# Edward-Sun/DIFUSCO

Measured on NVIDIA H100. Metric: TSP-500 graphs/sec, 50-step categorical denoise, higher is better.
Workload: dtype f32 (3-term bf16 split on wgmma, fp32 accumulate)

## Files before the change

### difusco_b200/_cabi.py

```python
import ctypes as C
import os

import numpy as np

HERE = os.path.dirname(os.path.abspath(__file__))
LIB_PATH = os.path.join(HERE, "libdifusco_b200.so")

DFB_OK, DFB_E_INVALID, DFB_E_CUDA, DFB_E_UNSUPPORTED, DFB_E_NOMEM = 0, -1, -2, -3, -4
CATEGORICAL, GAUSSIAN = 0, 1
EDGE_IMPL_TC, EDGE_IMPL_FP32, EDGE_IMPL_TC1 = 0, 1, 2
AGGREGATION = {"sum": 0, "mean": 1, "max": 2}

SYMBOLS = [
    "dfb_abi_version", "dfb_create", "dfb_destroy", "dfb_last_error", "dfb_set_aggregation",
    "dfb_set_edge_impl", "dfb_load_weights", "dfb_prepare_graph", "dfb_prepare_graph_instances", "dfb_set_points",
    "dfb_encoder_forward", "dfb_denoise_step", "dfb_denoise", "dfb_denoise_record", "dfb_denoise_host",
    "dfb_launch_count", "dfb_profile_begin", "dfb_profile_end", "dfb_debug_edge_gemm", "dfb_debug_gnn_layer",
    "dfb_debug_phase_cycles", "dfb_debug_watchdog", "dfb_knn_graph", "dfb_set_graph_capture",
    "dfb_set_phase_timing", "dfb_tsp_merge_sparse", "dfb_tsp_merge_order", "dfb_two_opt", "dfb_write_heatmap_txt",
]

_lib = None


def lib():
  global _lib
  if _lib is not None:
    return _lib
  if not os.path.exists(LIB_PATH):
    raise RuntimeError(
        f"{LIB_PATH} not found: build it with `python -m difusco_b200.build` "
        "(difusco_b200 has no fallback path; the CUDA library is the product)")
  L = C.CDLL(LIB_PATH)
  vp, i32, i64, u64, f32 = C.c_void_p, C.c_int, C.c_int64, C.c_uint64, C.c_float
  L.dfb_abi_version.restype = i32
  L.dfb_create.argtypes = [C.POINTER(vp), i32]
  L.dfb_destroy.argtypes = [vp]
  L.dfb_last_error.argtypes = [vp]
  L.dfb_last_error.restype = C.c_char_p
  L.dfb_set_aggregation.argtypes = [vp, i32]
  L.dfb_set_edge_impl.argtypes = [vp, i32]
  L.dfb_load_weights.argtypes = [vp, i32, i32, i32, i32, i32, C.POINTER(C.c_char_p), C.POINTER(vp),
                                 C.POINTER(i64)]
  L.dfb_prepare_graph.argtypes = [vp, vp, i64, i64, i32, vp]
  L.dfb_prepare_graph_instances.argtypes = [vp, vp, i64, i64, i32, C.POINTER(i64), vp]
  L.dfb_set_points.argtypes = [vp, vp, vp]
  L.dfb_encoder_forward.argtypes = [vp, vp, f32, vp, vp]
  L.dfb_denoise_step.argtypes = [vp, i32, vp, f32, C.POINTER(f32), i32, vp, u64, i32, vp, vp, vp, vp]
  L.dfb_denoise.argtypes = [vp, i32, vp, i32, C.POINTER(C.c_int32), C.POINTER(f32),
                            C.POINTER(C.c_int32), vp, u64, vp]
  L.dfb_denoise_record.argtypes = [vp, i32, vp, i32, C.POINTER(C.c_int32), C.POINTER(f32), C.POINTER(C.c_int32), vp,
                                   u64, i32, C.POINTER(C.c_int32), vp, vp, vp, vp]
  L.dfb_denoise_host.argtypes = [vp, i32, vp, vp, i64, i64, i32, vp, i32, C.POINTER(C.c_int32),
                                 C.POINTER(f32), C.POINTER(C.c_int32), u64, vp, vp]
  L.dfb_launch_count.argtypes = [vp]
  L.dfb_launch_count.restype = i64
  L.dfb_profile_begin.argtypes = [vp]
  L.dfb_profile_end.argtypes = [vp, C.POINTER(C.c_double), C.POINTER(i64)]
  L.dfb_debug_edge_gemm.argtypes = [vp, i32, vp, vp, vp]
  L.dfb_debug_gnn_layer.argtypes = [vp, i32, f32, vp, vp, vp]
  L.dfb_debug_phase_cycles.argtypes = [vp, C.POINTER(C.c_uint64)]
  L.dfb_debug_watchdog.argtypes = [vp, C.POINTER(C.c_int)]
  L.dfb_set_graph_capture.argtypes = [vp, i32]
  L.dfb_set_phase_timing.argtypes = [vp, i32]
  L.dfb_knn_graph.argtypes = [vp, vp, i64, i32, i64, vp, vp]
  L.dfb_tsp_merge_sparse.argtypes = [vp, i64, vp, vp, i64, i32, vp, C.POINTER(i64)]
  L.dfb_tsp_merge_order.argtypes = [i64, vp, i64, vp, C.POINTER(i64)]
  L.dfb_two_opt.argtypes = [vp, vp, i64, vp, i64, i64, C.POINTER(i64), vp]
  L.dfb_write_heatmap_txt.argtypes = [C.c_char_p, i64, vp]
  for name in SYMBOLS:
    fn = getattr(L, name)
    if fn.restype is C.c_int and name not in ("dfb_abi_version",):
      fn.restype = i32
  _lib = L
  return L


class DfbError(RuntimeError):
  pass


def _raise(code, msg):
  msg = msg.decode() if isinstance(msg, bytes) else msg
  if code == DFB_E_INVALID:
    raise ValueError(msg)
  if code == DFB_E_UNSUPPORTED:
    raise NotImplementedError(msg)
  if code == DFB_E_NOMEM:
    raise MemoryError(msg)
  raise DfbError(msg)


MERGE_COMPLETE, MERGE_INCOMPLETE, MERGE_AMBIGUOUS = 0, 1, 2


def tsp_merge_sparse(points, heat, edge_index, mode=0):
  points = np.ascontiguousarray(points, dtype=np.float64)
  heat = np.ascontiguousarray(heat, dtype=np.float32).reshape(-1)
  edge_index = np.ascontiguousarray(edge_index, dtype=np.int64)
  n = points.shape[0]
  if edge_index.ndim != 2 or edge_index.shape[0] != 2 or edge_index.shape[1] != heat.shape[0]:
    raise ValueError("edge_index must be (2, E) with one heat value per edge")
  tour = np.empty(n + 1, dtype=np.int64)
  it = C.c_int64(0)
  rc = lib().dfb_tsp_merge_sparse(points.ctypes.data, n, heat.ctypes.data, edge_index.ctypes.data, heat.shape[0],
                                  int(mode), tour.ctypes.data, C.byref(it))
  if rc < 0:
    _raise(rc, "dfb_tsp_merge_sparse: invalid argument (n >= 3, indices inside [0, n), mode 0/1)")
  return rc, tour, it.value


def tsp_merge_order(n, order):
  order = np.ascontiguousarray(order, dtype=np.int64).reshape(-1)
  tour = np.empty(n + 1, dtype=np.int64)
  it = C.c_int64(0)
  rc = lib().dfb_tsp_merge_order(int(n), order.ctypes.data, order.shape[0], tour.ctypes.data, C.byref(it))
  if rc < 0:
    _raise(rc, "dfb_tsp_merge_order: invalid argument or the order does not complete a tour")
  return tour, it.value


def write_heatmap_txt(path, matrix):
  m = np.ascontiguousarray(matrix, dtype=np.float64)
  if m.ndim != 2 or m.shape[0] != m.shape[1]:
    raise ValueError("matrix must be square")
  rc = lib().dfb_write_heatmap_txt(os.fsencode(path), m.shape[0], m.ctypes.data)
  if rc != DFB_OK:
    _raise(rc, f"dfb_write_heatmap_txt: cannot write {path}")


_DEVICE_CTX = {}


def device_context(device_index, prefer=None):
  ctx = _DEVICE_CTX.get(device_index)
  if ctx is None or getattr(ctx, "_h", None) is None:
    ctx = prefer if prefer is not None else Context(device_index)
    _DEVICE_CTX[device_index] = ctx
  return ctx


class Context(object):

  def __init__(self, device=0):
    L = lib()
    h = C.c_void_p()
    rc = L.dfb_create(C.byref(h), int(device))
    if rc != DFB_OK:
      _raise(rc, L.dfb_last_error(None))
    self._h = h
    self.device = int(device)
    self._keep = []

  def close(self):
    if getattr(self, "_h", None):
      lib().dfb_destroy(self._h)
      self._h = None

  def __del__(self):
    try:
      self.close()
    except Exception:
      pass

  def _ck(self, rc):
    if rc != DFB_OK:
      _raise(rc, lib().dfb_last_error(self._h))

  def load_weights(self, state_dict, n_layers, hidden_dim, out_channels, node_feature_only, consts=None):
    items = [(k, np.ascontiguousarray(v, dtype=np.float32)) for k, v in state_dict.items()]
    for k, v in (consts or {}).items():
      items.append((k, np.ascontiguousarray(v, dtype=np.float32)))
    n = len(items)
    names = (C.c_char_p * n)(*[k.encode() for k, _ in items])
    ptrs = (C.c_void_p * n)(*[v.ctypes.data for _, v in items])
    numels = (C.c_int64 * n)(*[v.size for _, v in items])
    self._ck(lib().dfb_load_weights(self._h, n_layers, hidden_dim, out_channels, int(bool(node_feature_only)),
                                    n, names, ptrs, numels))

  def set_aggregation(self, name):
    if name not in AGGREGATION:
      raise ValueError(f"unknown aggregation {name}")
    self._ck(lib().dfb_set_aggregation(self._h, AGGREGATION[name]))

  def set_edge_impl(self, impl):
    self._ck(lib().dfb_set_edge_impl(self._h, impl))

  def prepare_graph(self, edge_index_ptr, num_nodes, num_edges, gn_segments=1, stream=0):
    self._ck(lib().dfb_prepare_graph(self._h, edge_index_ptr, num_nodes, num_edges, gn_segments, stream))

  def prepare_graph_instances(self, edge_index_ptr, num_nodes, num_edges, node_ptr, stream=0):
    node_ptr = np.ascontiguousarray(node_ptr, dtype=np.int64)
    self._ck(lib().dfb_prepare_graph_instances(self._h, edge_index_ptr, num_nodes, num_edges, node_ptr.size - 1,
                                               node_ptr.ctypes.data_as(C.POINTER(C.c_int64)), stream))

  def set_points(self, points_ptr, stream=0):
    self._ck(lib().dfb_set_points(self._h, points_ptr, stream))

  def encoder_forward(self, xt_ptr, t, out_ptr, stream=0):
    self._ck(lib().dfb_encoder_forward(self._h, xt_ptr, float(t), out_ptr, stream))

  def denoise_step(self, diffusion, xt_in_ptr, t, consts, last, uniforms_ptr, seed, step_index, xt_out_ptr,
                   p_out_ptr=None, net_out_ptr=None, stream=0):
    c = (C.c_float * 4)(*[float(x) for x in consts])
    self._ck(lib().dfb_denoise_step(self._h, diffusion, xt_in_ptr, float(t), c, int(last), uniforms_ptr,
                                    int(seed) & 0xFFFFFFFFFFFFFFFF, int(step_index), xt_out_ptr, p_out_ptr,
                                    net_out_ptr, stream))

  @staticmethod
  def _sched_arrays(t1, consts, last):
    steps = len(t1)
    t1a = (C.c_int32 * steps)(*[int(x) for x in t1])
    ca = (C.c_float * (4 * steps))(*[float(x) for row in consts for x in row])
    la = (C.c_int32 * steps)(*[int(x) for x in last])
    return steps, t1a, ca, la

  def denoise(self, diffusion, xt_ptr, t1, consts, last, uniforms_ptr=None, seed=0, stream=0):
    steps, t1a, ca, la = self._sched_arrays(t1, consts, last)
    self._ck(lib().dfb_denoise(self._h, diffusion, xt_ptr, steps, t1a, ca, la, uniforms_ptr,
                               int(seed) & 0xFFFFFFFFFFFFFFFF, stream))

  def denoise_record(self, diffusion, xt_ptr, t1, consts, last, record_steps, rec_xt_ptr=None, rec_p_ptr=None,
                     rec_out_ptr=None, uniforms_ptr=None, seed=0, stream=0):
    steps, t1a, ca, la = self._sched_arrays(t1, consts, last)
    n_rec = len(record_steps)
    ra = (C.c_int32 * max(n_rec, 1))(*[int(x) for x in record_steps])
    self._ck(lib().dfb_denoise_record(self._h, diffusion, xt_ptr, steps, t1a, ca, la, uniforms_ptr,
                                      int(seed) & 0xFFFFFFFFFFFFFFFF, n_rec, ra, rec_xt_ptr, rec_p_ptr, rec_out_ptr,
                                      stream))

  def denoise_host(self, diffusion, points_ptr, edge_index_ptr, num_nodes, num_edges, gn_segments, xt0_ptr,
                   t1, consts, last, seed, heatmap_ptr, stream=0):
    steps, t1a, ca, la = self._sched_arrays(t1, consts, last)
    self._ck(lib().dfb_denoise_host(self._h, diffusion, points_ptr, edge_index_ptr, num_nodes, num_edges,
                                    gn_segments, xt0_ptr, steps, t1a, ca, la,
                                    int(seed) & 0xFFFFFFFFFFFFFFFF, heatmap_ptr, stream))

  def two_opt(self, points, tours, max_iterations, stream=0):
    points = np.ascontiguousarray(points, dtype=np.float64)
    tours = np.array(tours, dtype=np.int64, order="C", copy=True)
    if tours.ndim != 2 or tours.shape[1] != points.shape[0] + 1:
      raise ValueError("tours must be (batch, n + 1)")
    it = C.c_int64(0)
    self._ck(lib().dfb_two_opt(self._h, points.ctypes.data, points.shape[0], tours.ctypes.data, tours.shape[0],
                               int(max_iterations), C.byref(it), stream))
    return tours, it.value

  def knn_graph(self, points_ptr, num_nodes, k, node_offset, edge_index_ptr, stream=0):
    self._ck(lib().dfb_knn_graph(self._h, points_ptr, int(num_nodes), int(k), int(node_offset), edge_index_ptr, stream))

  def launch_count(self):
    return int(lib().dfb_launch_count(self._h))

  def profile_begin(self):
    self._ck(lib().dfb_profile_begin(self._h))

  def profile_end(self):
    ms, n = C.c_double(0), C.c_int64(0)
    self._ck(lib().dfb_profile_end(self._h, C.byref(ms), C.byref(n)))
    return ms.value, n.value

  def set_graph_capture(self, enabled):
    self._ck(lib().dfb_set_graph_capture(self._h, int(bool(enabled))))

  def debug_watchdog(self):
    out = (C.c_int * 4)()
    lib().dfb_debug_watchdog(self._h, out)
    return [int(x) for x in out]

  def set_phase_timing(self, enabled):
    self._ck(lib().dfb_set_phase_timing(self._h, int(bool(enabled))))

  def debug_phase_cycles(self):
    out = (C.c_uint64 * 32)()
    self._ck(lib().dfb_debug_phase_cycles(self._h, out))
    return [int(x) for x in out]

  def debug_edge_gemm(self, layer, e_in_ptr, acc_out_ptr, stream=0):
    self._ck(lib().dfb_debug_edge_gemm(self._h, layer, e_in_ptr, acc_out_ptr, stream))

  def debug_gnn_layer(self, layer, t, h_ptr, e_ptr, stream=0):
    self._ck(lib().dfb_debug_gnn_layer(self._h, int(layer), float(t), h_ptr, e_ptr, stream))
```

### difusco_b200/csrc/dfb_api.cu

```cuda
#include <cuda_runtime.h>
#include <math.h>
#include <stdio.h>
#include <stdlib.h>
#include <string.h>

#include <map>
#include <string>
#include <vector>

#include "../../include/difusco_b200.h"
#include "common.cuh"
#include "edge_layer_fp32.cuh"
#include "edge_layer_tc.cuh"
#include "kernels_small.cuh"
#include "knn.cuh"
#include "tsp_decode.cuh"

using namespace dfb;

static std::string g_create_error;

struct DevBuf {
  void* p = nullptr;
  size_t cap = 0;
  DevBuf() = default;
  DevBuf(const DevBuf&) = delete;
  DevBuf& operator=(const DevBuf&) = delete;
  ~DevBuf() { if (p) cudaFree(p); }
};

struct dfb_ctx {
  int device = 0;
  std::string err;
  bool weights_loaded = false;
  int L = 0, out_channels = 0, node_only = 0;
  int agg_mode = AGG_SUM;
  int edge_impl = DFB_EDGE_IMPL_TC;
  bool phase_timing = false;
  DevBuf wbuf, wbuf16, layers_dev;
  std::vector<LayerParams> layers;
  TimeParams tp{};
  HeadParams hp{};
  const float *Wt_node = nullptr, *b_node = nullptr, *Wt_edge = nullptr, *b_edge = nullptr;
  const float *dimt128 = nullptr, *dimt256 = nullptr;
  float* lut = nullptr;
  bool graph_ready = false, points_ready = false;
  GraphDev g{};
  GnSegments gseg{};
  int gn_blocks = 0;
  DevBuf d_row, d_col, d_perm, d_rowptr, d_grp_first, d_grp_pair, d_ei_stage, d_seg_start, d_seg_blk_first, d_gn_blk;
  DevBuf e, h, h0, uvab, uvab0, partials, feat, tvec, tvals, gn_part, gn_stats, d_points, d_xt, d_u;
  DevBuf opt_points, opt_tours, opt_pos, opt_dnext, opt_cand, opt_tiles, opt_state, opt_best;
  int tvec_steps_cap = 0;
  static constexpr int STAGE_SLOTS = 2, MAX_STEPS = 4096;
  float* h_tvals[STAGE_SLOTS] = {nullptr, nullptr};
  StepParams* h_steps[STAGE_SLOTS] = {nullptr, nullptr};
  cudaEvent_t stage_ev[STAGE_SLOTS] = {nullptr, nullptr};
  int stage_next = 0;
  DevBuf d_steps;
  uint64_t buf_gen = 0;
  bool capture_enabled = true;
  bool capture_broken = false;
  cudaGraphExec_t loop_exec = nullptr;
  cudaStream_t loop_stream = nullptr;
  cudaEvent_t loop_in = nullptr, loop_out = nullptr;
  struct LoopKey {
    uint64_t buf_gen = ~0ull;
    int steps = 0, diffusion = 0, impl = 0, agg = 0;
    bool timed = false;
    const void* uniforms = nullptr;
    bool operator==(const LoopKey& o) const {
      return buf_gen == o.buf_gen && steps == o.steps && diffusion == o.diffusion && impl == o.impl && agg == o.agg &&
             timed == o.timed && uniforms == o.uniforms;
    }
  } loop_key;
  int64_t loop_launches = 0;
  int64_t launches = 0;
  bool profiling = false;
  std::vector<cudaEvent_t> ev_pool;
  size_t ev_used = 0;
  TcState tc;

  ~dfb_ctx() {
    for (cudaEvent_t ev : ev_pool) cudaEventDestroy(ev);
    if (loop_exec) cudaGraphExecDestroy(loop_exec);
    if (loop_stream) cudaStreamDestroy(loop_stream);
    if (loop_in) cudaEventDestroy(loop_in);
    if (loop_out) cudaEventDestroy(loop_out);
    for (int i = 0; i < STAGE_SLOTS; ++i) {
      if (h_tvals[i]) cudaFreeHost(h_tvals[i]);
      if (h_steps[i]) cudaFreeHost(h_steps[i]);
      if (stage_ev[i]) cudaEventDestroy(stage_ev[i]);
    }
  }
};

#define FAIL(ctx, code, ...)                         \
  do {                                               \
    char _b[512];                                    \
    snprintf(_b, sizeof(_b), __VA_ARGS__);           \
    (ctx)->err = _b;                                 \
    return (code);                                   \
  } while (0)

#define CK(ctx, call)                                                                       \
  do {                                                                                      \
    cudaError_t _e = (call);                                                                \
    if (_e != cudaSuccess)                                                                  \
      FAIL(ctx, DFB_E_CUDA, "%s failed: %s (%s:%d)", #call, cudaGetErrorString(_e), __FILE__, __LINE__); \
  } while (0)

#define CKL(ctx)                                                                           \
  do {                                                                                      \
    (ctx)->launches++;                                                                      \
    cudaError_t _e = cudaGetLastError();                                                    \
    if (_e != cudaSuccess)                                                                  \
      FAIL(ctx, DFB_E_CUDA, "kernel launch failed: %s (%s:%d)", cudaGetErrorString(_e), __FILE__, __LINE__); \
  } while (0)

static int ensure(dfb_ctx* ctx, DevBuf& b, size_t bytes) {
  if (bytes <= b.cap) return DFB_OK;
  ctx->buf_gen++;
  if (b.p) cudaFree(b.p);
  b.p = nullptr;
  b.cap = 0;
  size_t want = bytes + (bytes >> 3);
  cudaError_t e = cudaMalloc(&b.p, want);
  if (e != cudaSuccess) {
    e = cudaMalloc(&b.p, bytes);
    want = bytes;
  }
  if (e != cudaSuccess) {
    cudaGetLastError();
    FAIL(ctx, DFB_E_NOMEM, "cudaMalloc(%zu bytes) failed: %s", bytes, cudaGetErrorString(e));
  }
  b.cap = want;
  return DFB_OK;
}
#define ENS(ctx, buf, bytes)                     \
  do {                                           \
    int _r = ensure(ctx, buf, bytes);            \
    if (_r) return _r;                           \
  } while (0)

static bool is_device_ptr(const void* p) {
  cudaPointerAttributes a;
  if (cudaPointerGetAttributes(&a, p) != cudaSuccess) {
    cudaGetLastError();
    return false;
  }
  return a.type == cudaMemoryTypeDevice || a.type == cudaMemoryTypeManaged;
}

extern "C" int dfb_abi_version(void) { return DFB_ABI_VERSION; }

extern "C" const char* dfb_last_error(const dfb_ctx* ctx) {
  return ctx ? ctx->err.c_str() : g_create_error.c_str();
}

extern "C" int dfb_create(dfb_ctx** out, int device) {
  if (!out) return DFB_E_INVALID;
  *out = nullptr;
  int n = 0;
  cudaError_t e = cudaGetDeviceCount(&n);
  if (e != cudaSuccess || n == 0) {
    g_create_error = std::string("no CUDA device: ") + cudaGetErrorString(e) +
                     " (difusco_b200 has no CPU fallback)";
    cudaGetLastError();
    return DFB_E_CUDA;
  }
  if (device < 0 || device >= n) {
    g_create_error = "device index out of range";
    return DFB_E_INVALID;
  }
  if ((e = cudaSetDevice(device)) != cudaSuccess) {
    g_create_error = std::string("cudaSetDevice: ") + cudaGetErrorString(e);
    return DFB_E_CUDA;
  }
  cudaDeviceProp prop;
  cudaGetDeviceProperties(&prop, device);
  if (prop.major != 9 || prop.minor != 0) {
    char b[160];
    snprintf(b, sizeof(b), "device %d is sm_%d%d; this library is built for sm_90a (H100) only", device,
             prop.major, prop.minor);
    g_create_error = b;
    return DFB_E_UNSUPPORTED;
  }
  dfb_ctx* ctx = new dfb_ctx();
  ctx->device = device;
  e = cudaFuncSetAttribute(k_edge_layer_fp32, cudaFuncAttributeMaxDynamicSharedMemorySize, EF_SMEM);
  if (e != cudaSuccess) {
    g_create_error = std::string("cudaFuncSetAttribute(fp32 edge kernel): ") + cudaGetErrorString(e);
    delete ctx;
    return DFB_E_CUDA;
  }
  int r = tc_init(&ctx->tc, prop.multiProcessorCount);
  if (r != 0) {
    g_create_error = "tensor-core edge kernel setup failed: " + ctx->tc.err;
    delete ctx;
    return DFB_E_CUDA;
  }
  for (int i = 0; i < dfb_ctx::STAGE_SLOTS; ++i) {
    if ((e = cudaHostAlloc((void**)&ctx->h_tvals[i], dfb_ctx::MAX_STEPS * sizeof(float), cudaHostAllocDefault)) != cudaSuccess ||
        (e = cudaHostAlloc((void**)&ctx->h_steps[i], dfb_ctx::MAX_STEPS * sizeof(StepParams), cudaHostAllocDefault)) != cudaSuccess ||
        (e = cudaEventCreateWithFlags(&ctx->stage_ev[i], cudaEventDisableTiming)) != cudaSuccess) {
      g_create_error = std::string("pinned staging: ") + cudaGetErrorString(e);
      delete ctx;
      return DFB_E_CUDA;
    }
  }
  if ((e = cudaStreamCreateWithFlags(&ctx->loop_stream, cudaStreamNonBlocking)) != cudaSuccess ||
      (e = cudaEventCreateWithFlags(&ctx->loop_in, cudaEventDisableTiming)) != cudaSuccess ||
      (e = cudaEventCreateWithFlags(&ctx->loop_out, cudaEventDisableTiming)) != cudaSuccess) {
    g_create_error = std::string("loop stream: ") + cudaGetErrorString(e);
    delete ctx;
    return DFB_E_CUDA;
  }
  {
    const char* cg = getenv("DFB_GRAPH_CAPTURE");
    if (cg && atoi(cg) == 0) ctx->capture_enabled = false;
  }
  *out = ctx;
  return DFB_OK;
}

extern "C" int dfb_destroy(dfb_ctx* ctx) {
  if (!ctx) return DFB_OK;
  cudaSetDevice(ctx->device);
  delete ctx;
  return DFB_OK;
}

extern "C" int dfb_set_edge_impl(dfb_ctx* ctx, int impl) {
  if (!ctx) return DFB_E_INVALID;
  if (impl != DFB_EDGE_IMPL_TC && impl != DFB_EDGE_IMPL_FP32 && impl != DFB_EDGE_IMPL_TC1) FAIL(ctx, DFB_E_INVALID, "unknown edge impl %d", impl);
  ctx->edge_impl = impl;
  return DFB_OK;
}

extern "C" int64_t dfb_launch_count(const dfb_ctx* ctx) { return ctx ? ctx->launches : 0; }

static uint16_t f2bf16_rn(float f) {
  uint32_t u;
  memcpy(&u, &f, 4);
  if ((u & 0x7fffffffu) > 0x7f800000u) return (uint16_t)((u >> 16) | 0x40);
  uint32_t r = u + 0x7fffu + ((u >> 16) & 1u);
  return (uint16_t)(r >> 16);
}
static float bf16_to_f(uint16_t h) {
  uint32_t u = (uint32_t)h << 16;
  float f;
  memcpy(&f, &u, 4);
  return f;
}

extern "C" int dfb_load_weights(dfb_ctx* ctx, int n_layers, int hidden_dim, int out_channels,
                                int node_feature_only, int n_tensors, const char* const* names,
                                const float* const* tensors, const int64_t* numels) {
  if (!ctx) return DFB_E_INVALID;
  CK(ctx, cudaSetDevice(ctx->device));
  if (hidden_dim != H) FAIL(ctx, DFB_E_UNSUPPORTED, "hidden_dim %d: kernels are specialised for 256", hidden_dim);
  if (n_layers < 1 || n_layers > 64) FAIL(ctx, DFB_E_INVALID, "n_layers %d out of range", n_layers);
  if (out_channels != 1 && out_channels != 2) FAIL(ctx, DFB_E_INVALID, "out_channels must be 1 or 2");
  std::map<std::string, std::pair<const float*, int64_t>> sd;
  for (int i = 0; i < n_tensors; ++i) {
    std::string k = names[i];
    if (k.rfind("model.", 0) == 0) k = k.substr(6);
    sd[k] = {tensors[i], numels[i]};
  }
  auto get = [&](const std::string& k, int64_t n, const float** out) -> int {
    auto it = sd.find(k);
    if (it == sd.end()) FAIL(ctx, DFB_E_INVALID, "state_dict key '%s' missing", k.c_str());
    if (it->second.second != n)
      FAIL(ctx, DFB_E_INVALID, "state_dict key '%s' has %lld elements, expected %lld", k.c_str(),
           (long long)it->second.second, (long long)n);
    *out = it->second.first;
    return DFB_OK;
  };
#define GET(k, n, out)                 \
  do {                                 \
    int _r = get(k, n, out);           \
    if (_r) return _r;                 \
  } while (0)

  const int L = n_layers;
  std::vector<float> arena;
  auto put = [&](size_t n) {
    size_t off = arena.size();
    arena.resize(off + ((n + 63) / 64) * 64, 0.0f);
    return off;
  };
  auto put_T = [&](const float* W, int out_f, int in_f) {
    size_t off = put((size_t)out_f * in_f);
    for (int o = 0; o < out_f; ++o)
      for (int i = 0; i < in_f; ++i) arena[off + (size_t)i * out_f + o] = W[(size_t)o * in_f + i];
    return off;
  };
  auto put_v = [&](const float* v, int n) {
    size_t off = put(n);
    memcpy(&arena[off], v, n * sizeof(float));
    return off;
  };
  struct LOff {
    size_t Wt_uvab, b_uvab, Wt_C, Wt_O, b_O, hg, hb, eg, eb, og, ob, Wt_tau, b_tau;
  };
  std::vector<LOff> lo(L);
  std::vector<uint16_t> arena16((size_t)w_arena_rows(L) * H);
  auto put16 = [&](const float* W, int row) {
    uint16_t* hi = &arena16[(size_t)row * H];
    for (int i = 0; i < H * H; ++i) {
      hi[i] = f2bf16_rn(W[i]);
      hi[W_LO_ROWS * H + i] = f2bf16_rn(W[i] - bf16_to_f(hi[i]));
    }
  };
  const float* p;
  for (int l = 0; l < L; ++l) {
    std::string pre = "layers." + std::to_string(l) + ".";
    const float *W[4], *b[4], *WC, *bC;
    const char* nm[4] = {"U", "V", "A", "B"};
    for (int q = 0; q < 4; ++q) {
      GET(pre + nm[q] + ".weight", H * H, &W[q]);
      GET(pre + nm[q] + ".bias", H, &b[q]);
    }
    GET(pre + "C.weight", H * H, &WC);
    GET(pre + "C.bias", H, &bC);
    lo[l].Wt_uvab = put((size_t)H * 4 * H);
    lo[l].b_uvab = put(4 * H);
    for (int q = 0; q < 4; ++q) {
      for (int o = 0; o < H; ++o) {
        for (int i = 0; i < H; ++i) arena[lo[l].Wt_uvab + (size_t)i * 4 * H + q * H + o] = W[q][(size_t)o * H + i];
        arena[lo[l].b_uvab + q * H + o] = b[q][o] + (q == 3 ? bC[o] : 0.0f);
      }
    }
    lo[l].Wt_C = put_T(WC, H, H);
    GET(pre + "norm_h.weight", H, &p); lo[l].hg = put_v(p, H);
    GET(pre + "norm_h.bias", H, &p);   lo[l].hb = put_v(p, H);
    GET(pre + "norm_e.weight", H, &p); lo[l].eg = put_v(p, H);
    GET(pre + "norm_e.bias", H, &p);   lo[l].eb = put_v(p, H);
    std::string po = "per_layer_out." + std::to_string(l) + ".";
    const float* WO;
    GET(po + "0.weight", H, &p); lo[l].og = put_v(p, H);
    GET(po + "0.bias", H, &p);   lo[l].ob = put_v(p, H);
    GET(po + "2.weight", H * H, &WO); lo[l].Wt_O = put_T(WO, H, H);
    GET(po + "2.bias", H, &p);   lo[l].b_O = put_v(p, H);
    std::string pt = "time_embed_layers." + std::to_string(l) + ".1.";
    GET(pt + "weight", H * TE, &p); lo[l].Wt_tau = put_T(p, H, TE);
    GET(pt + "bias", H, &p);        lo[l].b_tau = put_v(p, H);
    put16(WC, w_row_C(l));
    put16(WO, w_row_O(l));
    for (int q = 0; q < 4; ++q) put16(W[q], w_row_UVAB(l) + q * W_MAT_ROWS);
  }
  size_t o_node_W, o_node_b, o_edge_W, o_edge_b, o_t0W, o_t0b, o_t2W, o_t2b, o_gng, o_gnb, o_outW, o_outb;
  GET("node_embed.weight", H * H, &p); o_node_W = put_T(p, H, H); put16(p, w_row_embed(L, 1));
  GET("node_embed.bias", H, &p);       o_node_b = put_v(p, H);
  GET("edge_embed.weight", H * H, &p); o_edge_W = put_T(p, H, H); put16(p, w_row_embed(L, 0));
  GET("edge_embed.bias", H, &p);       o_edge_b = put_v(p, H);
  GET("time_embed.0.weight", TE * H, &p); o_t0W = put_T(p, TE, H);
  GET("time_embed.0.bias", TE, &p);       o_t0b = put_v(p, TE);
  GET("time_embed.2.weight", TE * TE, &p); o_t2W = put_T(p, TE, TE);
  GET("time_embed.2.bias", TE, &p);        o_t2b = put_v(p, TE);
  GET("out.0.weight", H, &p); o_gng = put_v(p, H);
  GET("out.0.bias", H, &p);   o_gnb = put_v(p, H);
  GET("out.2.weight", out_channels * H, &p); o_outW = put_v(p, out_channels * H);
  GET("out.2.bias", out_channels, &p);       o_outb = put_v(p, out_channels);

  size_t o_freqs = put(TE), o_d128 = put(TE), o_d256 = put(H), o_lut = put(2 * H);
  auto it = sd.find("__const.time_freqs");
  for (int m = 0; m < TE; ++m)
    arena[o_freqs + m] = (it != sd.end() && it->second.second == TE)
                             ? it->second.first[m]
                             : expf((-9.210340371976184f * (float)m) / (float)TE);
  it = sd.find("__const.dimt_pos");
  for (int m = 0; m < TE; ++m)
    arena[o_d128 + m] = (it != sd.end() && it->second.second == TE)
                            ? it->second.first[m]
                            : powf(10000.0f, (2.0f * (float)(m / 2)) / (float)TE);
  it = sd.find("__const.dimt_scalar");
  for (int m = 0; m < H; ++m)
    arena[o_d256 + m] = (it != sd.end() && it->second.second == H)
                            ? it->second.first[m]
                            : powf(10000.0f, (2.0f * (float)(m / 2)) / (float)H);

  ENS(ctx, ctx->wbuf, arena.size() * sizeof(float));
  ENS(ctx, ctx->wbuf16, arena16.size() * sizeof(uint16_t));
  ENS(ctx, ctx->layers_dev, L * sizeof(LayerParams));
  CK(ctx, cudaMemcpy(ctx->wbuf.p, arena.data(), arena.size() * sizeof(float), cudaMemcpyHostToDevice));
  CK(ctx, cudaMemcpy(ctx->wbuf16.p, arena16.data(), arena16.size() * sizeof(uint16_t), cudaMemcpyHostToDevice));
  const float* base = (const float*)ctx->wbuf.p;
  ctx->layers.resize(L);
  for (int l = 0; l < L; ++l) {
    LayerParams& lp = ctx->layers[l];
    lp.Wt_uvab = base + lo[l].Wt_uvab; lp.b_uvab = base + lo[l].b_uvab;
    lp.Wt_C = base + lo[l].Wt_C; lp.Wt_O = base + lo[l].Wt_O; lp.b_O = base + lo[l].b_O;
    lp.ln_h_g = base + lo[l].hg; lp.ln_h_b = base + lo[l].hb;
    lp.ln_e_g = base + lo[l].eg; lp.ln_e_b = base + lo[l].eb;
    lp.ln_o_g = base + lo[l].og; lp.ln_o_b = base + lo[l].ob;
    lp.Wt_tau = base + lo[l].Wt_tau; lp.b_tau = base + lo[l].b_tau;
  }
  CK(ctx, cudaMemcpy(ctx->layers_dev.p, ctx->layers.data(), L * sizeof(LayerParams), cudaMemcpyHostToDevice));
  ctx->Wt_node = base + o_node_W; ctx->b_node = base + o_node_b;
  ctx->Wt_edge = base + o_edge_W; ctx->b_edge = base + o_edge_b;
  ctx->tp.freqs = base + o_freqs; ctx->tp.Wt0 = base + o_t0W; ctx->tp.b0 = base + o_t0b;
  ctx->tp.Wt2 = base + o_t2W;     ctx->tp.b2 = base + o_t2b;
  ctx->hp.gn_g = base + o_gng; ctx->hp.gn_b = base + o_gnb; ctx->hp.W = base + o_outW; ctx->hp.b = base + o_outb;
  ctx->hp.out_channels = out_channels;
  ctx->dimt128 = base + o_d128; ctx->dimt256 = base + o_d256;
  ctx->lut = (float*)ctx->wbuf.p + o_lut;
  ctx->L = L; ctx->out_channels = out_channels; ctx->node_only = node_feature_only;

  int r = tc_bind_weights(&ctx->tc, (const uint16_t*)ctx->wbuf16.p, L);
  if (r) FAIL(ctx, DFB_E_CUDA, "tensor-map setup failed: %s", ctx->tc.err.c_str());

  if (!node_feature_only) {
    ENS(ctx, ctx->feat, (size_t)LIN_ROWS * H * sizeof(float));
    float x01[2] = {0.0f, 1.0f};
    ENS(ctx, ctx->tvals, 4096 * sizeof(float));
    CK(ctx, cudaMemcpy(ctx->tvals.p, x01, sizeof(x01), cudaMemcpyHostToDevice));
    k_scalar_features<<<2, H>>>((const float*)ctx->tvals.p, nullptr, ctx->dimt256, (float*)ctx->feat.p, 2);
    CKL(ctx);
    k_linear<<<dim3(1, 1), 256>>>((const float*)ctx->feat.p, ctx->Wt_edge, ctx->b_edge, ctx->lut, 2, H);
    CKL(ctx);
    CK(ctx, cudaDeviceSynchronize());
  }
  ctx->weights_loaded = true;
  ctx->buf_gen++;
  ctx->points_ready = false;
  return DFB_OK;
}

extern "C" int dfb_set_aggregation(dfb_ctx* ctx, int mode) {
  if (!ctx) return DFB_E_INVALID;
  if (mode < AGG_SUM || mode > AGG_MAX) FAIL(ctx, DFB_E_INVALID, "unknown aggregation %d", mode);
  ctx->agg_mode = mode;
  return DFB_OK;
}

static int prepare_graph(dfb_ctx* ctx, const int64_t* edge_index, int64_t V64, int64_t E64, int gn_segments,
                         int n_inst, const int64_t* node_ptr, cudaStream_t st) {
  if (!ctx) return DFB_E_INVALID;
  CK(ctx, cudaSetDevice(ctx->device));
  if (!ctx->weights_loaded) FAIL(ctx, DFB_E_INVALID, "dfb_load_weights must be called first");
  if (V64 <= 0 || E64 <= 0 || V64 > 0x7fffffff / 4 || E64 > 0x7ffffff0)
    FAIL(ctx, DFB_E_INVALID, "bad graph size V=%lld E=%lld", (long long)V64, (long long)E64);
  const int V = (int)V64, E = (int)E64;
  const int R = ctx->node_only ? V : E;
  if (!node_ptr) {
    if (gn_segments < 1) FAIL(ctx, DFB_E_INVALID, "gn_segments must be >= 1");
    if (R % gn_segments) FAIL(ctx, DFB_E_INVALID, "gn_segments %d does not divide %d rows", gn_segments, R);
  } else {
    if (n_inst < 1) FAIL(ctx, DFB_E_INVALID, "n_instances %d < 1", n_inst);
    if (node_ptr[0] != 0 || node_ptr[n_inst] != V64)
      FAIL(ctx, DFB_E_INVALID, "node_ptr must run from 0 to num_nodes %lld (got %lld .. %lld)", (long long)V64,
           (long long)node_ptr[0], (long long)node_ptr[n_inst]);
    for (int i = 0; i < n_inst; ++i)
      if (node_ptr[i + 1] <= node_ptr[i])
        FAIL(ctx, DFB_E_INVALID, "node_ptr must be strictly increasing (instance %d: %lld after %lld)", i,
             (long long)node_ptr[i + 1], (long long)node_ptr[i]);
  }
  std::vector<int64_t> stage;
  const int64_t* ei = edge_index;
  if (is_device_ptr(edge_index)) {
    stage.resize((size_t)2 * E);
    CK(ctx, cudaMemcpyAsync(stage.data(), edge_index, (size_t)2 * E * sizeof(int64_t), cudaMemcpyDeviceToHost, st));
    CK(ctx, cudaStreamSynchronize(st));
    ei = stage.data();
  }
  const int64_t* row64 = ei;
  const int64_t* col64 = ei + E;
  std::vector<int> inst;
  if (node_ptr) {
    inst.resize(V);
    for (int i = 0; i < n_inst; ++i)
      for (int64_t v = node_ptr[i]; v < node_ptr[i + 1]; ++v) inst[v] = i;
  }
  std::vector<int> rowptr((size_t)V + 1, 0);
  bool sorted = true;
  for (int s = 0; s < E; ++s) {
    int64_t r = row64[s], c = col64[s];
    if (r < 0 || r >= V || c < 0 || c >= V)
      FAIL(ctx, DFB_E_INVALID, "edge %d = (%lld,%lld) out of range for %d nodes", s, (long long)r, (long long)c, V);
    if (node_ptr && inst[r] != inst[c])
      FAIL(ctx, DFB_E_INVALID, "edge %d = (%lld,%lld) joins instances %d and %d", s, (long long)r, (long long)c,
           inst[r], inst[c]);
    rowptr[(size_t)r + 1]++;
    if (s && r < row64[s - 1]) sorted = false;
  }
  for (int i = 0; i < V; ++i) rowptr[i + 1] += rowptr[i];
  const int S = node_ptr ? n_inst : gn_segments;
  std::vector<int> seg_start((size_t)S + 1), blk_first((size_t)S + 1);
  for (int i = 0; i <= S; ++i) {
    if (!node_ptr) seg_start[i] = (int)((int64_t)R / S * i);
    else seg_start[i] = ctx->node_only ? (int)node_ptr[i] : rowptr[node_ptr[i]];
  }
  for (int i = 0; i < S; ++i)
    if (seg_start[i + 1] == seg_start[i])
      FAIL(ctx, DFB_E_INVALID, "instance %d (nodes %lld..%lld) has no edges: its GroupNorm would be over zero rows", i,
           (long long)node_ptr[i], (long long)node_ptr[i + 1] - 1);
  std::vector<int2> gn_blk;
  for (int i = 0; i < S; ++i) {
    blk_first[i] = (int)gn_blk.size();
    for (int r0 = seg_start[i]; r0 < seg_start[i + 1]; r0 += GN_ROWS_PER_BLOCK) gn_blk.push_back(make_int2(i, r0));
  }
  blk_first[S] = (int)gn_blk.size();
  const int nb = (int)gn_blk.size();

  std::vector<int> row(E), col(E), perm;
  if (sorted) {
    for (int s = 0; s < E; ++s) {
      row[s] = (int)row64[s];
      col[s] = (int)col64[s];
    }
  } else {
    perm.resize(E);
    std::vector<int> cur(rowptr.begin(), rowptr.end() - 1);
    for (int s = 0; s < E; ++s) {
      int pos = cur[row64[s]]++;
      perm[pos] = s;
      row[pos] = (int)row64[s];
      col[pos] = (int)col64[s];
    }
  }
  const int nG = (E + GROUP - 1) / GROUP;
  std::vector<int> gfirst(nG), gpair((size_t)nG + 1);
  int np = 0;
  for (int gI = 0; gI < nG; ++gI) {
    int s0 = gI * GROUP, s1 = std::min(E, s0 + GROUP) - 1;
    gfirst[gI] = row[s0];
    gpair[gI] = np;
    np += row[s1] - row[s0] + 1;
  }
  gpair[nG] = np;

  ENS(ctx, ctx->d_row, (size_t)E * 4);
  ENS(ctx, ctx->d_col, (size_t)E * 4);
  ENS(ctx, ctx->d_rowptr, ((size_t)V + 1) * 4);
  ENS(ctx, ctx->d_grp_first, (size_t)nG * 4);
  ENS(ctx, ctx->d_grp_pair, ((size_t)nG + 1) * 4);
  CK(ctx, cudaMemcpyAsync(ctx->d_row.p, row.data(), (size_t)E * 4, cudaMemcpyHostToDevice, st));
  CK(ctx, cudaMemcpyAsync(ctx->d_col.p, col.data(), (size_t)E * 4, cudaMemcpyHostToDevice, st));
  CK(ctx, cudaMemcpyAsync(ctx->d_rowptr.p, rowptr.data(), ((size_t)V + 1) * 4, cudaMemcpyHostToDevice, st));
  CK(ctx, cudaMemcpyAsync(ctx->d_grp_first.p, gfirst.data(), (size_t)nG * 4, cudaMemcpyHostToDevice, st));
  CK(ctx, cudaMemcpyAsync(ctx->d_grp_pair.p, gpair.data(), ((size_t)nG + 1) * 4, cudaMemcpyHostToDevice, st));
  if (!sorted) {
    ENS(ctx, ctx->d_perm, (size_t)E * 4);
    CK(ctx, cudaMemcpyAsync(ctx->d_perm.p, perm.data(), (size_t)E * 4, cudaMemcpyHostToDevice, st));
  }
  ENS(ctx, ctx->d_seg_start, ((size_t)S + 1) * 4);
  ENS(ctx, ctx->d_seg_blk_first, ((size_t)S + 1) * 4);
  ENS(ctx, ctx->d_gn_blk, (size_t)nb * sizeof(int2));
  CK(ctx, cudaMemcpyAsync(ctx->d_seg_start.p, seg_start.data(), ((size_t)S + 1) * 4, cudaMemcpyHostToDevice, st));
  CK(ctx, cudaMemcpyAsync(ctx->d_seg_blk_first.p, blk_first.data(), ((size_t)S + 1) * 4, cudaMemcpyHostToDevice, st));
  CK(ctx, cudaMemcpyAsync(ctx->d_gn_blk.p, gn_blk.data(), (size_t)nb * sizeof(int2), cudaMemcpyHostToDevice, st));
  CK(ctx, cudaStreamSynchronize(st));
  GraphDev& g = ctx->g;
  g.V = V; g.E = E;
  g.row = (const int*)ctx->d_row.p; g.col = (const int*)ctx->d_col.p;
  g.perm = sorted ? nullptr : (const int*)ctx->d_perm.p;
  g.rowptr = (const int*)ctx->d_rowptr.p;
  g.n_groups = nG; g.grp_first = (const int*)ctx->d_grp_first.p; g.grp_pair = (const int*)ctx->d_grp_pair.p;
  g.n_pairs = np;
  ctx->gseg.n_segs = S;
  ctx->gseg.start = (const int*)ctx->d_seg_start.p;
  ctx->gseg.blk_first = (const int*)ctx->d_seg_blk_first.p;
  ctx->gseg.blk = (const int2*)ctx->d_gn_blk.p;
  ctx->gn_blocks = nb;

  ENS(ctx, ctx->e, (size_t)E * H * sizeof(float));
  ENS(ctx, ctx->h, (size_t)V * H * sizeof(float));
  ENS(ctx, ctx->h0, (size_t)V * H * sizeof(float));
  ENS(ctx, ctx->uvab, (size_t)V * 4 * H * sizeof(float));
  ENS(ctx, ctx->uvab0, (size_t)V * 4 * H * sizeof(float));
  ENS(ctx, ctx->partials, (size_t)np * H * sizeof(float));
  const size_t feat_rows = 65536;
  ENS(ctx, ctx->feat, feat_rows * H * sizeof(float));
  ENS(ctx, ctx->gn_part, std::max((size_t)nb, (size_t)1024) * 32 * 2 * sizeof(double));
  ENS(ctx, ctx->gn_stats, (size_t)S * 32 * 2 * sizeof(float));
  ENS(ctx, ctx->d_xt, (size_t)std::max(V, E) * sizeof(float));
  ctx->graph_ready = true;
  ctx->buf_gen++;
  ctx->points_ready = false;
  return DFB_OK;
}

extern "C" int dfb_prepare_graph(dfb_ctx* ctx, const int64_t* edge_index, int64_t num_nodes, int64_t num_edges,
                                 int gn_segments, void* stream) {
  return prepare_graph(ctx, edge_index, num_nodes, num_edges, gn_segments, 0, nullptr, (cudaStream_t)stream);
}

extern "C" int dfb_prepare_graph_instances(dfb_ctx* ctx, const int64_t* edge_index, int64_t num_nodes,
                                           int64_t num_edges, int n_instances, const int64_t* node_ptr, void* stream) {
  if (ctx && !node_ptr) FAIL(ctx, DFB_E_INVALID, "node_ptr is required");
  return prepare_graph(ctx, edge_index, num_nodes, num_edges, 0, n_instances, node_ptr, (cudaStream_t)stream);
}

struct EdgeImpl { bool fp32; int nwg; };
static EdgeImpl edge_impl(const dfb_ctx* ctx) {
  return {ctx->edge_impl == DFB_EDGE_IMPL_FP32, ctx->edge_impl == DFB_EDGE_IMPL_TC1 ? 1 : 2};
}

static int linear_rows(dfb_ctx* ctx, const float* X, const float* Wt, int w_row, const float* b, float* Y, int R, int N,
                       cudaStream_t st) {
  if (edge_impl(ctx).fp32) {
    dim3 grid((R + LIN_ROWS - 1) / LIN_ROWS, N / 256);
    k_linear<<<grid, 256, 0, st>>>(X, Wt, b, Y, R, N);
    CKL(ctx);
    return DFB_OK;
  }
  if (tc_launch_linear(&ctx->tc, X, Y, b, R, N / H, w_row, st))
    FAIL(ctx, DFB_E_CUDA, "tensor-core linear: %s", ctx->tc.err.c_str());
  ctx->launches++;
  return DFB_OK;
}

static int node_linears(dfb_ctx* ctx, int l, const float* h, float* uvab, int V, cudaStream_t st) {
  const LayerParams& lp = ctx->layers[l];
  return linear_rows(ctx, h, lp.Wt_uvab, w_row_UVAB(l), lp.b_uvab, uvab, V, 4 * H, st);
}

static int embed_rows(dfb_ctx* ctx, int which, const float* X, float* Y, int R, cudaStream_t st) {
  return linear_rows(ctx, X, which ? ctx->Wt_node : ctx->Wt_edge, w_row_embed(ctx->L, which),
                     which ? ctx->b_node : ctx->b_edge, Y, R, H, st);
}

extern "C" int dfb_set_points(dfb_ctx* ctx, const float* points, void* stream_) {
  if (!ctx) return DFB_E_INVALID;
  cudaStream_t st = (cudaStream_t)stream_;
  CK(ctx, cudaSetDevice(ctx->device));
  if (!ctx->graph_ready) FAIL(ctx, DFB_E_INVALID, "dfb_prepare_graph must be called first");
  if (ctx->node_only) FAIL(ctx, DFB_E_INVALID, "dfb_set_points is for the TSP encoder (node_feature_only=0)");
  const int V = ctx->g.V;
  const float* dp = points;
  if (!is_device_ptr(points)) {
    ENS(ctx, ctx->d_points, (size_t)V * 2 * sizeof(float));
    CK(ctx, cudaMemcpyAsync(ctx->d_points.p, points, (size_t)V * 2 * sizeof(float), cudaMemcpyHostToDevice, st));
    dp = (const float*)ctx->d_points.p;
  }
  const int CH = 65536;
  for (int v0 = 0; v0 < V; v0 += CH) {
    int n = std::min(CH, V - v0);
    k_pos_features<<<n, H, 0, st>>>(dp + (size_t)v0 * 2, ctx->dimt128, (float*)ctx->feat.p, n);
    CKL(ctx);
    int r = embed_rows(ctx, 1, (const float*)ctx->feat.p, (float*)ctx->h0.p + (size_t)v0 * H, n, st);
    if (r) return r;
  }
  int r = node_linears(ctx, 0, (const float*)ctx->h0.p, (float*)ctx->uvab0.p, V, st);
  if (r) return r;
  ctx->points_ready = true;
  return DFB_OK;
}

static int launch_edge_layer(dfb_ctx* ctx, int l, float* e, const float* uvab, const float* tvec_edge, int write_e,
                             int e_zero, const float* xt_for_lut, cudaStream_t st) {
  cudaEvent_t ev0 = nullptr, ev1 = nullptr;
  if (ctx->profiling) {
    if (ctx->ev_used + 2 > ctx->ev_pool.size()) {
      for (int i = 0; i < 256; ++i) {
        cudaEvent_t ev;
        CK(ctx, cudaEventCreate(&ev));
        ctx->ev_pool.push_back(ev);
      }
    }
    ev0 = ctx->ev_pool[ctx->ev_used++];
    ev1 = ctx->ev_pool[ctx->ev_used++];
    CK(ctx, cudaEventRecord(ev0, st));
  }
  const EdgeImpl impl = edge_impl(ctx);
  if (impl.fp32) {
    if (e_zero) CK(ctx, cudaMemsetAsync(e, 0, (size_t)ctx->g.E * H * sizeof(float), st));
    if (xt_for_lut) {
      k_lut_expand<<<(ctx->g.E + 3) / 4, 256, 0, st>>>(xt_for_lut, ctx->g.perm, ctx->lut, e, ctx->g.E);
      CKL(ctx);
    }
    k_edge_layer_fp32<<<ctx->g.n_groups, 256, EF_SMEM, st>>>(e, uvab, (float*)ctx->partials.p,
                                                            ctx->g, ctx->layers[l], tvec_edge, write_e,
                                                            ctx->agg_mode);
    CKL(ctx);
  } else {
    if (tc_launch_edge_layer(&ctx->tc, l, e, uvab, (float*)ctx->partials.p, ctx->g, ctx->layers[l],
                             tvec_edge, write_e, e_zero, xt_for_lut, ctx->lut, ctx->agg_mode, impl.nwg,
                             ctx->phase_timing, nullptr, st))
      FAIL(ctx, DFB_E_CUDA, "tensor-core edge layer: %s", ctx->tc.err.c_str());
    ctx->launches++;
  }
  if (ctx->profiling) CK(ctx, cudaEventRecord(ev1, st));
  return DFB_OK;
}

static int run_layer(dfb_ctx* ctx, int l, float* h, float* e, const float* uv0, const float* tv, int e_zero,
                     const float* xt_lut, cudaStream_t st) {
  const int L = ctx->L;
  const float* uv = uv0;
  if (!uv) {
    int r = node_linears(ctx, l, h, (float*)ctx->uvab.p, ctx->g.V, st);
    if (r) return r;
    uv = (const float*)ctx->uvab.p;
  }
  const int write_e = !(ctx->node_only && l == L - 1);
  int r = launch_edge_layer(ctx, l, e, uv, ctx->node_only ? nullptr : tv, write_e, e_zero, xt_lut, st);
  if (r) return r;
  if (ctx->node_only || l < L - 1) {
    k_node_update<<<(ctx->g.V + 7) / 8, 256, 0, st>>>(h, uv, (const float*)ctx->partials.p, ctx->g,
                                                      ctx->layers[l].ln_h_g, ctx->layers[l].ln_h_b,
                                                      ctx->node_only ? tv : nullptr, ctx->agg_mode);
    CKL(ctx);
  }
  return DFB_OK;
}

static int run_forward(dfb_ctx* ctx, const float* xt, const float* tvec, bool binary_xt, PosteriorArgs pa,
                       cudaStream_t st) {
  const GraphDev& g = ctx->g;
  const int V = g.V, E = g.E;
  float* h = (float*)ctx->h.p;
  float* e = (float*)ctx->e.p;
  const float* xt_lut = nullptr;
  int e_zero = 0;
  if (!ctx->node_only) {
    if (!ctx->points_ready) FAIL(ctx, DFB_E_INVALID, "dfb_set_points must be called before a TSP forward");
    CK(ctx, cudaMemcpyAsync(h, ctx->h0.p, (size_t)V * H * sizeof(float), cudaMemcpyDeviceToDevice, st));
    if (binary_xt) {
      xt_lut = xt;
    } else {
      const int CH = 65536;
      for (int s0 = 0; s0 < E; s0 += CH) {
        int n = std::min(CH, E - s0);
        k_scalar_features<<<n, H, 0, st>>>(g.perm ? xt : xt + s0, g.perm ? g.perm + s0 : nullptr, ctx->dimt256,
                                           (float*)ctx->feat.p, n);
        CKL(ctx);
        int r = embed_rows(ctx, 0, (const float*)ctx->feat.p, e + (size_t)s0 * H, n, st);
        if (r) return r;
      }
    }
  } else {
    const int CH = 65536;
    for (int v0 = 0; v0 < V; v0 += CH) {
      int n = std::min(CH, V - v0);
      k_scalar_features<<<n, H, 0, st>>>(xt + v0, nullptr, ctx->dimt256, (float*)ctx->feat.p, n);
      CKL(ctx);
      int r = embed_rows(ctx, 1, (const float*)ctx->feat.p, h + (size_t)v0 * H, n, st);
      if (r) return r;
    }
    e_zero = 1;
  }
  for (int l = 0; l < ctx->L; ++l) {
    const bool first = l == 0;
    int r = run_layer(ctx, l, h, e, (first && !ctx->node_only) ? (const float*)ctx->uvab0.p : nullptr,
                      tvec + (size_t)l * H, first ? e_zero : 0, first ? xt_lut : nullptr, st);
    if (r) return r;
  }
  const float* Z = ctx->node_only ? h : e;
  const int R = ctx->node_only ? V : E;
  k_gn_partial<<<ctx->gn_blocks, 256, 0, st>>>(Z, ctx->gseg, (double*)ctx->gn_part.p);
  CKL(ctx);
  k_gn_final<<<dim3(ctx->gseg.n_segs, 32), 256, 0, st>>>((const double*)ctx->gn_part.p, Z, ctx->gseg,
                                                         (float*)ctx->gn_stats.p);
  CKL(ctx);
  k_head<<<(R + 255) / 256, 256, 0, st>>>(Z, R, ctx->gseg, (const float*)ctx->gn_stats.p,
                                      ctx->node_only ? nullptr : g.perm, ctx->hp, pa);
  CKL(ctx);
  return DFB_OK;
}

static int stage_acquire(dfb_ctx* ctx, int* slot) {
  *slot = ctx->stage_next;
  ctx->stage_next = (ctx->stage_next + 1) % dfb_ctx::STAGE_SLOTS;
  CK(ctx, cudaEventSynchronize(ctx->stage_ev[*slot]));
  return DFB_OK;
}

static int compute_tvecs(dfb_ctx* ctx, int slot, int S, cudaStream_t st) {
  ENS(ctx, ctx->tvals, std::max<size_t>(4096, (size_t)S) * sizeof(float));
  ENS(ctx, ctx->tvec, (size_t)S * ctx->L * H * sizeof(float));
  CK(ctx, cudaMemcpyAsync(ctx->tvals.p, ctx->h_tvals[slot], (size_t)S * sizeof(float), cudaMemcpyHostToDevice, st));
  k_time_vectors<<<S, 256, 0, st>>>((const float*)ctx->tvals.p, ctx->tp, (const LayerParams*)ctx->layers_dev.p,
                                    ctx->L, (float*)ctx->tvec.p);
  CKL(ctx);
  return DFB_OK;
}

extern "C" int dfb_encoder_forward(dfb_ctx* ctx, const float* xt, float t, float* out, void* stream_) {
  if (!ctx) return DFB_E_INVALID;
  cudaStream_t st = (cudaStream_t)stream_;
  CK(ctx, cudaSetDevice(ctx->device));
  if (!ctx->graph_ready) FAIL(ctx, DFB_E_INVALID, "dfb_prepare_graph must be called first");
  int slot;
  int r = stage_acquire(ctx, &slot);
  if (r) return r;
  ctx->h_tvals[slot][0] = t;
  r = compute_tvecs(ctx, slot, 1, st);
  if (r) return r;
  CK(ctx, cudaEventRecord(ctx->stage_ev[slot], st));
  PosteriorArgs pa{};
  pa.mode = HEAD_FORWARD;
  pa.net_out = out;
  return run_forward(ctx, xt, (const float*)ctx->tvec.p, false, pa, st);
}

static int step_args(dfb_ctx* ctx, int diffusion_type, const float* consts, int last, PosteriorArgs* pa) {
  if (diffusion_type == DFB_DIFFUSION_CATEGORICAL) {
    if (ctx->out_channels != 2) FAIL(ctx, DFB_E_INVALID, "categorical diffusion needs out_channels == 2");
    pa->mode = HEAD_CATEGORICAL;
  } else if (diffusion_type == DFB_DIFFUSION_GAUSSIAN) {
    if (ctx->out_channels != 1) FAIL(ctx, DFB_E_INVALID, "gaussian diffusion needs out_channels == 1");
    pa->mode = HEAD_GAUSSIAN;
  } else {
    FAIL(ctx, DFB_E_INVALID, "Unknown diffusion type %d", diffusion_type);
  }
  if (consts)
    for (int i = 0; i < 4; ++i) pa->c[i] = consts[i];
  pa->last = last;
  return DFB_OK;
}

extern "C" int dfb_denoise_step(dfb_ctx* ctx, int diffusion_type, const float* xt_in, float t,
                                const float* consts, int last, const float* uniforms, uint64_t seed,
                                int step_index, float* xt_out, float* p_out, float* net_out, void* stream_) {
  if (!ctx) return DFB_E_INVALID;
  cudaStream_t st = (cudaStream_t)stream_;
  CK(ctx, cudaSetDevice(ctx->device));
  if (!ctx->graph_ready) FAIL(ctx, DFB_E_INVALID, "dfb_prepare_graph must be called first");
  PosteriorArgs pa{};
  int r = step_args(ctx, diffusion_type, consts, last, &pa);
  if (r) return r;
  int slot;
  r = stage_acquire(ctx, &slot);
  if (r) return r;
  ctx->h_tvals[slot][0] = t;
  r = compute_tvecs(ctx, slot, 1, st);
  if (r) return r;
  CK(ctx, cudaEventRecord(ctx->stage_ev[slot], st));
  pa.xt_in = xt_in; pa.uniforms = uniforms; pa.seed = seed; pa.step = (unsigned)step_index;
  pa.xt_out = xt_out; pa.p_out = p_out; pa.net_out = net_out;
  return run_forward(ctx, xt_in, (const float*)ctx->tvec.p, diffusion_type == DFB_DIFFUSION_CATEGORICAL, pa, st);
}

static int enqueue_loop(dfb_ctx* ctx, int diffusion_type, float* xt, int steps, const float* uniforms, cudaStream_t st) {
  const size_t N = ctx->node_only ? ctx->g.V : ctx->g.E;
  for (int i = 0; i < steps; ++i) {
    PosteriorArgs pa{};
    int r = step_args(ctx, diffusion_type, nullptr, 0, &pa);
    if (r) return r;
    pa.sp = (const StepParams*)ctx->d_steps.p + i;
    pa.xt_in = xt; pa.xt_out = xt;
    pa.uniforms = uniforms ? uniforms + (size_t)i * N : nullptr;
    r = run_forward(ctx, xt, (const float*)ctx->tvec.p + (size_t)i * ctx->L * H,
                    diffusion_type == DFB_DIFFUSION_CATEGORICAL, pa, st);
    if (r) return r;
  }
  return DFB_OK;
}

extern "C" int dfb_denoise(dfb_ctx* ctx, int diffusion_type, float* xt, int steps, const int32_t* t1,
                           const float* consts, const int32_t* last_flags, const float* uniforms,
                           uint64_t seed, void* stream_) {
  return dfb_denoise_record(ctx, diffusion_type, xt, steps, t1, consts, last_flags, uniforms, seed, 0, nullptr,
                            nullptr, nullptr, nullptr, stream_);
}

extern "C" int dfb_denoise_record(dfb_ctx* ctx, int diffusion_type, float* xt, int steps, const int32_t* t1,
                                  const float* consts, const int32_t* last_flags, const float* uniforms,
                                  uint64_t seed, int n_record, const int32_t* record_steps, float* rec_xt,
                                  float* rec_p, float* rec_out, void* stream_) {
  if (!ctx) return DFB_E_INVALID;
  cudaStream_t st = (cudaStream_t)stream_;
  CK(ctx, cudaSetDevice(ctx->device));
  if (!ctx->graph_ready) FAIL(ctx, DFB_E_INVALID, "dfb_prepare_graph must be called first");
  if (steps < 1 || steps > dfb_ctx::MAX_STEPS) FAIL(ctx, DFB_E_INVALID, "steps %d out of range", steps);
  if (!ctx->node_only && !ctx->points_ready) FAIL(ctx, DFB_E_INVALID, "dfb_set_points must be called before a TSP forward");
  {
    PosteriorArgs chk{};
    int r = step_args(ctx, diffusion_type, nullptr, 0, &chk);
    if (r) return r;
  }
  if (n_record < 0) FAIL(ctx, DFB_E_INVALID, "n_record %d < 0", n_record);
  if (n_record > 0) {
    if (!record_steps) FAIL(ctx, DFB_E_INVALID, "n_record > 0 needs record_steps");
    if (!rec_xt && !rec_p && !rec_out) FAIL(ctx, DFB_E_INVALID, "n_record > 0 with no record buffer");
    if (rec_p && diffusion_type != DFB_DIFFUSION_CATEGORICAL)
      FAIL(ctx, DFB_E_INVALID, "rec_p is the categorical posterior: not defined for gaussian diffusion");
    for (int j = 0; j < n_record; ++j) {
      if (record_steps[j] < 0 || record_steps[j] >= steps)
        FAIL(ctx, DFB_E_INVALID, "record step %d outside [0, %d)", record_steps[j], steps);
      if (j > 0 && record_steps[j] <= record_steps[j - 1])
        FAIL(ctx, DFB_E_INVALID, "record steps must be strictly increasing (%d after %d)", record_steps[j],
             record_steps[j - 1]);
    }
  }
  int slot;
  int r = stage_acquire(ctx, &slot);
  if (r) return r;
  const size_t N = ctx->node_only ? ctx->g.V : ctx->g.E;
  for (int i = 0, j = 0; i < steps; ++i) {
    ctx->h_tvals[slot][i] = (float)t1[i];
    StepParams& sp = ctx->h_steps[slot][i];
    for (int k = 0; k < 4; ++k) sp.c[k] = consts[4 * i + k];
    sp.last = last_flags[i];
    sp.step = (unsigned)i;
    sp.seed = seed;
    sp.rec_xt = sp.rec_p = sp.rec_out = nullptr;
    if (j < n_record && record_steps[j] == i) {
      if (rec_xt) sp.rec_xt = rec_xt + (size_t)j * N;
      if (rec_p) sp.rec_p = rec_p + (size_t)j * N;
      if (rec_out) sp.rec_out = rec_out + (size_t)j * N * ctx->out_channels;
      ++j;
    }
  }
  ENS(ctx, ctx->d_steps, (size_t)dfb_ctx::MAX_STEPS * sizeof(StepParams));
  r = compute_tvecs(ctx, slot, steps, st);
  if (r) return r;
  CK(ctx, cudaMemcpyAsync(ctx->d_steps.p, ctx->h_steps[slot], (size_t)steps * sizeof(StepParams), cudaMemcpyHostToDevice, st));
  CK(ctx, cudaEventRecord(ctx->stage_ev[slot], st));
  float* x = (float*)ctx->d_xt.p;
  if (xt != x) CK(ctx, cudaMemcpyAsync(x, xt, N * sizeof(float), cudaMemcpyDeviceToDevice, st));

  const bool want_graph = ctx->capture_enabled && !ctx->capture_broken && !ctx->profiling;
  if (want_graph) {
    dfb_ctx::LoopKey key;
    key.buf_gen = ctx->buf_gen; key.steps = steps; key.diffusion = diffusion_type; key.impl = ctx->edge_impl;
    key.agg = ctx->agg_mode; key.timed = ctx->phase_timing; key.uniforms = uniforms;
    if (!ctx->loop_exec || !(ctx->loop_key == key)) {
      if (ctx->loop_exec) {
        cudaGraphExecDestroy(ctx->loop_exec);
        ctx->loop_exec = nullptr;
      }
      const int64_t l0 = ctx->launches;
      cudaGraph_t graph = nullptr;
      cudaError_t ce = cudaStreamBeginCapture(ctx->loop_stream, cudaStreamCaptureModeThreadLocal);
      if (ce == cudaSuccess) {
        r = enqueue_loop(ctx, diffusion_type, x, steps, uniforms, ctx->loop_stream);
        ce = cudaStreamEndCapture(ctx->loop_stream, &graph);
        if (r == DFB_OK && ce == cudaSuccess) ce = cudaGraphInstantiate(&ctx->loop_exec, graph, 0);
        if (graph) cudaGraphDestroy(graph);
      }
      ctx->loop_launches = ctx->launches - l0;
      ctx->launches = l0;
      if (r != DFB_OK || ce != cudaSuccess || !ctx->loop_exec) {
        cudaGetLastError();
        ctx->loop_exec = nullptr;
        ctx->capture_broken = true;
        if (r != DFB_OK) return r;
      } else {
        ctx->loop_key = key;
      }
    }
  }
  if (want_graph && ctx->loop_exec) {
    CK(ctx, cudaEventRecord(ctx->loop_in, st));
    CK(ctx, cudaStreamWaitEvent(ctx->loop_stream, ctx->loop_in, 0));
    CK(ctx, cudaGraphLaunch(ctx->loop_exec, ctx->loop_stream));
    CK(ctx, cudaEventRecord(ctx->loop_out, ctx->loop_stream));
    CK(ctx, cudaStreamWaitEvent(st, ctx->loop_out, 0));
    ctx->launches += ctx->loop_launches;
  } else {
    r = enqueue_loop(ctx, diffusion_type, x, steps, uniforms, st);
    if (r) return r;
  }
  if (xt != x) CK(ctx, cudaMemcpyAsync(xt, x, N * sizeof(float), cudaMemcpyDeviceToDevice, st));
  return DFB_OK;
}

extern "C" int dfb_set_graph_capture(dfb_ctx* ctx, int enabled) {
  if (!ctx) return DFB_E_INVALID;
  ctx->capture_enabled = enabled != 0;
  ctx->capture_broken = false;
  return DFB_OK;
}

extern "C" int dfb_set_phase_timing(dfb_ctx* ctx, int enabled) {
  if (!ctx) return DFB_E_INVALID;
  ctx->phase_timing = enabled != 0;
  return DFB_OK;
}

extern "C" int dfb_denoise_host(dfb_ctx* ctx, int diffusion_type, const float* points,
                                const int64_t* edge_index, int64_t V, int64_t E, int gn_segments,
                                const float* xt0, int steps, const int32_t* t1, const float* consts,
                                const int32_t* last_flags, uint64_t seed, float* heatmap_out, void* stream_) {
  if (!ctx) return DFB_E_INVALID;
  cudaStream_t st = (cudaStream_t)stream_;
  CK(ctx, cudaSetDevice(ctx->device));
  int r = dfb_prepare_graph(ctx, edge_index, V, E, gn_segments, st);
  if (r) return r;
  if (!ctx->node_only) {
    if (!points) FAIL(ctx, DFB_E_INVALID, "points required for TSP");
    r = dfb_set_points(ctx, points, st);
    if (r) return r;
  }
  const size_t N = ctx->node_only ? (size_t)V : (size_t)E;
  CK(ctx, cudaMemcpyAsync(ctx->d_xt.p, xt0, N * sizeof(float), cudaMemcpyHostToDevice, st));
  r = dfb_denoise(ctx, diffusion_type, (float*)ctx->d_xt.p, steps, t1, consts, last_flags, nullptr, seed, st);
  if (r) return r;
  CK(ctx, cudaMemcpyAsync(heatmap_out, ctx->d_xt.p, N * sizeof(float), cudaMemcpyDeviceToHost, st));
  CK(ctx, cudaStreamSynchronize(st));
  return DFB_OK;
}

extern "C" int dfb_profile_begin(dfb_ctx* ctx) {
  if (!ctx) return DFB_E_INVALID;
  ctx->profiling = true;
  ctx->ev_used = 0;
  return DFB_OK;
}
extern "C" int dfb_profile_end(dfb_ctx* ctx, double* ms, int64_t* n) {
  if (!ctx) return DFB_E_INVALID;
  CK(ctx, cudaSetDevice(ctx->device));
  CK(ctx, cudaDeviceSynchronize());
  double tot = 0.0;
  for (size_t i = 0; i + 1 < ctx->ev_used; i += 2) {
    float t = 0.f;
    CK(ctx, cudaEventElapsedTime(&t, ctx->ev_pool[i], ctx->ev_pool[i + 1]));
    tot += t;
  }
  if (ms) *ms = tot;
  if (n) *n = (int64_t)(ctx->ev_used / 2);
  ctx->profiling = false;
  ctx->ev_used = 0;
  return DFB_OK;
}

extern "C" int dfb_debug_edge_gemm(dfb_ctx* ctx, int layer, const float* e_in, float* acc_out, void* stream_) {
  if (!ctx) return DFB_E_INVALID;
  cudaStream_t st = (cudaStream_t)stream_;
  CK(ctx, cudaSetDevice(ctx->device));
  if (!ctx->graph_ready) FAIL(ctx, DFB_E_INVALID, "dfb_prepare_graph must be called first");
  if (layer < 0 || layer >= ctx->L) FAIL(ctx, DFB_E_INVALID, "layer out of range");
  if (tc_launch_edge_layer(&ctx->tc, layer, const_cast<float*>(e_in), (const float*)ctx->uvab.p,
                           (float*)ctx->partials.p, ctx->g, ctx->layers[layer], nullptr, 0, 0, nullptr, ctx->lut, AGG_SUM,
                           edge_impl(ctx).nwg, false, acc_out, st))
    FAIL(ctx, DFB_E_CUDA, "tensor-core edge layer: %s", ctx->tc.err.c_str());
  ctx->launches++;
  return DFB_OK;
}

extern "C" int dfb_debug_gnn_layer(dfb_ctx* ctx, int layer, float t, float* h, float* e, void* stream_) {
  if (!ctx) return DFB_E_INVALID;
  cudaStream_t st = (cudaStream_t)stream_;
  CK(ctx, cudaSetDevice(ctx->device));
  if (!ctx->graph_ready) FAIL(ctx, DFB_E_INVALID, "dfb_prepare_graph must be called first");
  if (layer < 0 || layer >= ctx->L) FAIL(ctx, DFB_E_INVALID, "layer %d out of range for %d layers", layer, ctx->L);
  if (!is_device_ptr(h) || !is_device_ptr(e)) FAIL(ctx, DFB_E_INVALID, "h and e must be device pointers");
  int slot;
  int r = stage_acquire(ctx, &slot);
  if (r) return r;
  ctx->h_tvals[slot][0] = t;
  r = compute_tvecs(ctx, slot, 1, st);
  if (r) return r;
  CK(ctx, cudaEventRecord(ctx->stage_ev[slot], st));
  return run_layer(ctx, layer, h, e, nullptr, (const float*)ctx->tvec.p + (size_t)layer * H, 0, nullptr, st);
}

extern "C" int dfb_debug_phase_cycles(dfb_ctx* ctx, unsigned long long* out) {
  if (!ctx || !out) return DFB_E_INVALID;
  CK(ctx, cudaSetDevice(ctx->device));
  CK(ctx, cudaDeviceSynchronize());
  CK(ctx, cudaMemcpy(out, ctx->tc.phase_cycles, 32 * sizeof(unsigned long long), cudaMemcpyDeviceToHost));
  CK(ctx, cudaMemset(ctx->tc.phase_cycles, 0, 32 * sizeof(unsigned long long)));
  return DFB_OK;
}

extern "C" int dfb_debug_watchdog(dfb_ctx* ctx, int* out) {
  if (!ctx || !out || !ctx->tc.error_host) return DFB_E_INVALID;
  for (int i = 0; i < 4; ++i) out[i] = ((volatile int*)ctx->tc.error_host)[i];
  return DFB_OK;
}

extern "C" int dfb_knn_graph(dfb_ctx* ctx, const double* points, int64_t num_nodes, int k, int64_t node_offset,
                             int64_t* edge_index, void* stream_) {
  if (!ctx) return DFB_E_INVALID;
  cudaStream_t st = (cudaStream_t)stream_;
  CK(ctx, cudaSetDevice(ctx->device));
  if (num_nodes < 1 || k < 1 || k > num_nodes) FAIL(ctx, DFB_E_INVALID, "bad kNN size N=%lld K=%d", (long long)num_nodes, k);
  if ((size_t)num_nodes * sizeof(double) > 200 * 1024) FAIL(ctx, DFB_E_UNSUPPORTED, "kNN graph: N=%lld exceeds the shared-memory brute-force limit (25600)", (long long)num_nodes);
  const size_t smem = (size_t)num_nodes * sizeof(double) + (size_t)(num_nodes + 31) / 32 * sizeof(unsigned);
  if (!is_device_ptr(edge_index)) FAIL(ctx, DFB_E_INVALID, "edge_index must be a device pointer");
  const double* dp = points;
  if (!is_device_ptr(points)) {
    for (int64_t i = 0; i < 2 * num_nodes; ++i)
      if (!std::isfinite(points[i])) FAIL(ctx, DFB_E_INVALID, "kNN graph: non-finite coordinate of node %lld", (long long)(i / 2));
    ENS(ctx, ctx->d_points, (size_t)num_nodes * 2 * sizeof(double));
    CK(ctx, cudaMemcpyAsync(ctx->d_points.p, points, (size_t)num_nodes * 2 * sizeof(double), cudaMemcpyHostToDevice, st));
    dp = (const double*)ctx->d_points.p;
  }
  CK(ctx, cudaFuncSetAttribute(k_knn_bruteforce, cudaFuncAttributeMaxDynamicSharedMemorySize, (int)smem));
  k_knn_bruteforce<<<(int)num_nodes, 256, smem, st>>>(dp, (int)num_nodes, k, (long long*)edge_index, (long long)node_offset);
  CKL(ctx);
  return DFB_OK;
}

extern "C" int dfb_tsp_merge_sparse(const double* points, int64_t n, const float* heat, const int64_t* edge_index, int64_t E,
                                    int mode, int64_t* tour, int64_t* merge_iterations) {
  if (!points || !heat || !edge_index || !tour || !merge_iterations || n < 3 || n > 0x7fffffff / 2 || E < 0 || (mode != 0 && mode != 1))
    return DFB_E_INVALID;
  int r = tspmerge::merge_sparse(points, (int)n, heat, edge_index, E, mode, tour, merge_iterations);
  return r < 0 ? DFB_E_INVALID : r;
}

extern "C" int dfb_tsp_merge_order(int64_t n, const int64_t* order, int64_t count, int64_t* tour, int64_t* merge_iterations) {
  if (!order || !tour || !merge_iterations || n < 3 || n > 0x7fffffff / 2 || count < 0) return DFB_E_INVALID;
  int r = tspmerge::merge_order((int)n, order, count, tour, merge_iterations);
  return r < 0 ? DFB_E_INVALID : r;
}

extern "C" int dfb_two_opt(dfb_ctx* ctx, const double* points, int64_t n, int64_t* tours, int64_t batch, int64_t max_iterations,
                           int64_t* iterations_out, void* stream_) {
  if (!ctx) return DFB_E_INVALID;
  cudaStream_t st = (cudaStream_t)stream_;
  CK(ctx, cudaSetDevice(ctx->device));
  if (!points || !tours || !iterations_out) FAIL(ctx, DFB_E_INVALID, "two_opt: null argument");
  if (n < 3 || n > 46340 || batch < 1 || batch > 65535) FAIL(ctx, DFB_E_INVALID, "two_opt: bad size n=%lld batch=%lld (n in [3, 46340], batch in [1, 65535])", (long long)n, (long long)batch);
  const int N = (int)n, B = (int)batch;
  bool finite = true;
  for (int64_t k = 0; k < batch * (n + 1); ++k) {
    if (tours[k] < 0 || tours[k] >= n) FAIL(ctx, DFB_E_INVALID, "two_opt: tour entry %lld out of range", (long long)tours[k]);
    finite = finite && std::isfinite(points[2 * tours[k]]) && std::isfinite(points[2 * tours[k] + 1]);
  }
  if (!finite) {
    *iterations_out = 0;
    return DFB_OK;
  }
  const int T = (N + TWOOPT_TILE - 1) / TWOOPT_TILE;
  std::vector<int2> tiles;
  for (int a = 0; a < T; ++a)
    for (int b = a; b < T; ++b) tiles.push_back(make_int2(a, b));
  const int ntiles = (int)tiles.size();
  ENS(ctx, ctx->opt_points, (size_t)N * 2 * sizeof(double));
  ENS(ctx, ctx->opt_tours, (size_t)B * (N + 1) * sizeof(long long));
  ENS(ctx, ctx->opt_pos, (size_t)B * (N + 1) * 2 * sizeof(double));
  ENS(ctx, ctx->opt_dnext, (size_t)B * N * sizeof(double));
  ENS(ctx, ctx->opt_cand, (size_t)B * ntiles * sizeof(TwoOptCand));
  ENS(ctx, ctx->opt_tiles, (size_t)ntiles * sizeof(int2));
  ENS(ctx, ctx->opt_state, sizeof(TwoOptState));
  ENS(ctx, ctx->opt_best, (size_t)B * sizeof(TwoOptCand));
  double* d_points = (double*)ctx->opt_points.p;
  long long* d_tours = (long long*)ctx->opt_tours.p;
  double* d_pos = (double*)ctx->opt_pos.p;
  double* d_dnext = (double*)ctx->opt_dnext.p;
  TwoOptCand* d_cand = (TwoOptCand*)ctx->opt_cand.p;
  int2* d_tiles = (int2*)ctx->opt_tiles.p;
  TwoOptState* d_state = (TwoOptState*)ctx->opt_state.p;
  CK(ctx, cudaMemcpyAsync(d_points, points, (size_t)N * 2 * sizeof(double), cudaMemcpyHostToDevice, st));
  CK(ctx, cudaMemcpyAsync(d_tours, tours, (size_t)B * (N + 1) * sizeof(long long), cudaMemcpyHostToDevice, st));
  CK(ctx, cudaMemcpyAsync(d_tiles, tiles.data(), (size_t)ntiles * sizeof(int2), cudaMemcpyHostToDevice, st));
  CK(ctx, cudaMemsetAsync(d_state, 0, sizeof(TwoOptState), st));
  k_twoopt_init<<<dim3((N + 256) / 256, B), 256, 0, st>>>(d_points, d_tours, d_pos, d_dnext, N);
  CKL(ctx);
  TwoOptState hs{};
  int chunk = 8;
  while (true) {
    for (int c = 0; c < chunk; ++c) {
      k_twoopt_eval<<<dim3(ntiles, B), 256, 0, st>>>(d_pos, d_dnext, d_tiles, d_cand, d_state, N, ntiles);
      CKL(ctx);
      k_twoopt_apply<<<1, 1024, 0, st>>>(d_tours, d_pos, d_dnext, d_cand, d_state, (TwoOptCand*)ctx->opt_best.p, N, B, ntiles,
                                         (long long)max_iterations);
      CKL(ctx);
    }
    CK(ctx, cudaMemcpyAsync(&hs, d_state, sizeof(hs), cudaMemcpyDeviceToHost, st));
    CK(ctx, cudaStreamSynchronize(st));
    if (hs.done) break;
    if (chunk < 64) chunk *= 2;
  }
  CK(ctx, cudaMemcpyAsync(tours, d_tours, (size_t)B * (N + 1) * sizeof(long long), cudaMemcpyDeviceToHost, st));
  CK(ctx, cudaStreamSynchronize(st));
  *iterations_out = hs.iterations;
  return DFB_OK;
}

extern "C" int dfb_write_heatmap_txt(const char* path, int64_t n, const double* matrix) {
  if (!path || !matrix || n < 1) return DFB_E_INVALID;
  FILE* f = fopen(path, "wb");
  if (!f) return DFB_E_INVALID;
  std::vector<char> line((size_t)n * 28 + 2);
  bool ok = fprintf(f, "%lld\n", (long long)n) > 0;
  for (int64_t r = 0; r < n && ok; ++r) {
    char* w = line.data();
    const double* row = matrix + r * n;
    for (int64_t c = 0; c < n; ++c) {
      if (c) *w++ = ' ';
      double x = row[c];
      if (x == 0.0 && !std::signbit(x)) {
        memcpy(w, "0.000000", 8);
        w += 8;
      } else {
        const int k = snprintf(w, 27, "%.6f", x);
        if (k < 0 || k > 26) {
          fclose(f);
          return DFB_E_INVALID;
        }
        w += k;
      }
    }
    *w++ = '\n';
    ok = fwrite(line.data(), 1, (size_t)(w - line.data()), f) == (size_t)(w - line.data());
  }
  ok = (fclose(f) == 0) && ok;
  return ok ? DFB_OK : DFB_E_INVALID;
}
```

### difusco_b200/csrc/edge_layer_tc.cuh

```cuda
#pragma once
#include <cuda.h>
#include <cuda_bf16.h>
#include <cuda_runtime.h>

#include <stdlib.h>

#include <string>

#include "common.cuh"
#include "edge_layer_fp32.cuh"

namespace dfb {

constexpr int WG_ROWS = 64;
constexpr int TC_KCH = 64;
constexpr int TC_B_BYTES = 256 * 128;
constexpr int TC_A_CHUNK = WG_ROWS * 128;
constexpr int TC_A_BYTES = 8 * TC_A_CHUNK;
constexpr int CONV_BATCH = 16;
constexpr int E4_BATCH = 16;

constexpr int W_LO_ROWS = H;
constexpr int W_MAT_ROWS = 2 * W_LO_ROWS;
constexpr int W_LAYER_ROWS = 6 * W_MAT_ROWS;
__host__ __device__ constexpr int w_row_C(int l) { return l * W_LAYER_ROWS; }
__host__ __device__ constexpr int w_row_O(int l) { return w_row_C(l) + W_MAT_ROWS; }
__host__ __device__ constexpr int w_row_UVAB(int l) { return w_row_C(l) + 2 * W_MAT_ROWS; }
__host__ __device__ constexpr int w_row_embed(int L, int which) { return L * W_LAYER_ROWS + which * W_MAT_ROWS; }
__host__ __device__ constexpr int w_arena_rows(int L) { return w_row_embed(L, 2); }

template <int NWG>
struct TcCfg {
  static_assert(NWG == 1 || NWG == 2, "one or two consumer warpgroups");
  static constexpr int TILE = NWG * WG_ROWS;
  static constexpr int THREADS = (NWG + 1) * 128;
  static constexpr int NSTAGE = (NWG == 1) ? 3 : 2;
  static constexpr int OFF_B = NWG * TC_A_BYTES;
  static constexpr int OFF_PRM = OFF_B + NSTAGE * TC_B_BYTES;
  static constexpr int OFF_ROW = OFF_PRM + 6 * H * 4;
  static constexpr int OFF_SRC = OFF_ROW + TILE * 4;
  static constexpr int OFF_BAR = OFF_SRC + TILE * 8;
  static constexpr int SMEM_BYTES = OFF_BAR + 2 * NSTAGE * 8;
  static constexpr int SMEM_ALLOC = SMEM_BYTES + 1024;
  static_assert(SMEM_ALLOC <= 232448, "shared memory budget (227 KB per block)");
};

struct TcParams {
  float* e;
  const float* uvab;
  float* partials;
  GraphDev g;
  LayerParams lp;
  const float* tvec;
  const float* xt_lut;
  const float* lut;
  const float* zero_row;
  float* debug_acc;
  const float* lin_in;
  float* lin_out;
  const float* lin_bias;
  int lin_rows;
  int lin_nb;
  int lin_w_row;
  int* error_flag;
  unsigned long long* phase_cycles;
  int write_e, e_zero, agg_mode;
  int w_row_base;
  int n_tiles;
};

__device__ __forceinline__ uint32_t smem_u32(const void* p) { return (uint32_t)__cvta_generic_to_shared(p); }

__device__ __forceinline__ void mbar_init(uint64_t* bar, uint32_t count) {
  asm volatile("mbarrier.init.shared::cta.b64 [%0], %1;" ::"r"(smem_u32(bar)), "r"(count) : "memory");
}
__device__ __forceinline__ void mbar_arrive(uint64_t* bar) {
  asm volatile("mbarrier.arrive.shared::cta.b64 _, [%0];" ::"r"(smem_u32(bar)) : "memory");
}
__device__ __forceinline__ void mbar_arrive_expect_tx(uint64_t* bar, uint32_t bytes) {
  asm volatile("mbarrier.arrive.expect_tx.shared::cta.b64 _, [%0], %1;" ::"r"(smem_u32(bar)), "r"(bytes) : "memory");
}
__device__ __forceinline__ void mbar_wait(uint64_t* bar, uint32_t parity, int* error_flag, int code) {
  const uint32_t addr = smem_u32(bar);
  uint32_t ok = 0;
#pragma unroll 1
  for (uint32_t spin = 0;; ++spin) {
    asm volatile(
        "{\n .reg .pred p;\n mbarrier.try_wait.parity.shared::cta.b64 p, [%1], %2, %3;\n selp.u32 %0, 1, 0, p;\n}"
        : "=r"(ok)
        : "r"(addr), "r"(parity), "r"(20000u)
        : "memory");
    if (ok) return;
    if (spin > 400000u) {
      if (error_flag) {
        error_flag[1] = (int)blockIdx.x;
        error_flag[2] = (int)parity;
        error_flag[3] = (int)threadIdx.x;
        atomicExch(error_flag, code);
      }
      __threadfence_system();
      __trap();
    }
  }
}
__device__ __forceinline__ void tma_load_2d(uint32_t dst, const CUtensorMap* map, uint64_t* bar, int c0, int c1) {
  asm volatile(
      "cp.async.bulk.tensor.2d.shared::cluster.global.mbarrier::complete_tx::bytes [%0], [%1, {%3, %4}], [%2];"
      ::"r"(dst), "l"(reinterpret_cast<uint64_t>(map)), "r"(smem_u32(bar)), "r"(c0), "r"(c1)
      : "memory");
}
__device__ __forceinline__ void fence_proxy_async() { asm volatile("fence.proxy.async.shared::cta;" ::: "memory"); }

__device__ __forceinline__ uint64_t wgmma_desc_sw128(uint32_t smem_addr) {
  return (uint64_t)((smem_addr >> 4) & 0x3fffu) | (1ull << 16) | (64ull << 32) | (1ull << 62);
}
__device__ __forceinline__ void wgmma_fence() { asm volatile("wgmma.fence.sync.aligned;" ::: "memory"); }
__device__ __forceinline__ void wgmma_commit() { asm volatile("wgmma.commit_group.sync.aligned;" ::: "memory"); }
template <int N>
__device__ __forceinline__ void wgmma_wait() { asm volatile("wgmma.wait_group.sync.aligned %0;" ::"n"(N) : "memory"); }
__device__ __forceinline__ void acc_fence(float (&d)[128]) {
#pragma unroll
  for (int i = 0; i < 128; ++i) asm volatile("" : "+f"(d[i])::"memory");
}
__device__ __forceinline__ void wgmma_bf16(float (&d)[128], uint64_t da, uint64_t db, uint32_t scale_d) {
  asm volatile(
      "{\n .reg .pred p;\n setp.ne.b32 p, %130, 0;\n"
      "wgmma.mma_async.sync.aligned.m64n256k16.f32.bf16.bf16 "
      "{%0, %1, %2, %3, %4, %5, %6, %7, %8, %9, %10, %11, %12, %13, %14, %15, "
      "%16, %17, %18, %19, %20, %21, %22, %23, %24, %25, %26, %27, %28, %29, %30, %31, "
      "%32, %33, %34, %35, %36, %37, %38, %39, %40, %41, %42, %43, %44, %45, %46, %47, "
      "%48, %49, %50, %51, %52, %53, %54, %55, %56, %57, %58, %59, %60, %61, %62, %63, "
      "%64, %65, %66, %67, %68, %69, %70, %71, %72, %73, %74, %75, %76, %77, %78, %79, "
      "%80, %81, %82, %83, %84, %85, %86, %87, %88, %89, %90, %91, %92, %93, %94, %95, "
      "%96, %97, %98, %99, %100, %101, %102, %103, %104, %105, %106, %107, %108, %109, %110, %111, "
      "%112, %113, %114, %115, %116, %117, %118, %119, %120, %121, %122, %123, %124, %125, %126, %127}, "
      "%128, %129, p, 1, 1, 0, 0;\n}"
      : "+f"(d[0]), "+f"(d[1]), "+f"(d[2]), "+f"(d[3]), "+f"(d[4]), "+f"(d[5]), "+f"(d[6]), "+f"(d[7]),
        "+f"(d[8]), "+f"(d[9]), "+f"(d[10]), "+f"(d[11]), "+f"(d[12]), "+f"(d[13]), "+f"(d[14]), "+f"(d[15]),
        "+f"(d[16]), "+f"(d[17]), "+f"(d[18]), "+f"(d[19]), "+f"(d[20]), "+f"(d[21]), "+f"(d[22]), "+f"(d[23]),
        "+f"(d[24]), "+f"(d[25]), "+f"(d[26]), "+f"(d[27]), "+f"(d[28]), "+f"(d[29]), "+f"(d[30]), "+f"(d[31]),
        "+f"(d[32]), "+f"(d[33]), "+f"(d[34]), "+f"(d[35]), "+f"(d[36]), "+f"(d[37]), "+f"(d[38]), "+f"(d[39]),
        "+f"(d[40]), "+f"(d[41]), "+f"(d[42]), "+f"(d[43]), "+f"(d[44]), "+f"(d[45]), "+f"(d[46]), "+f"(d[47]),
        "+f"(d[48]), "+f"(d[49]), "+f"(d[50]), "+f"(d[51]), "+f"(d[52]), "+f"(d[53]), "+f"(d[54]), "+f"(d[55]),
        "+f"(d[56]), "+f"(d[57]), "+f"(d[58]), "+f"(d[59]), "+f"(d[60]), "+f"(d[61]), "+f"(d[62]), "+f"(d[63]),
        "+f"(d[64]), "+f"(d[65]), "+f"(d[66]), "+f"(d[67]), "+f"(d[68]), "+f"(d[69]), "+f"(d[70]), "+f"(d[71]),
        "+f"(d[72]), "+f"(d[73]), "+f"(d[74]), "+f"(d[75]), "+f"(d[76]), "+f"(d[77]), "+f"(d[78]), "+f"(d[79]),
        "+f"(d[80]), "+f"(d[81]), "+f"(d[82]), "+f"(d[83]), "+f"(d[84]), "+f"(d[85]), "+f"(d[86]), "+f"(d[87]),
        "+f"(d[88]), "+f"(d[89]), "+f"(d[90]), "+f"(d[91]), "+f"(d[92]), "+f"(d[93]), "+f"(d[94]), "+f"(d[95]),
        "+f"(d[96]), "+f"(d[97]), "+f"(d[98]), "+f"(d[99]), "+f"(d[100]), "+f"(d[101]), "+f"(d[102]), "+f"(d[103]),
        "+f"(d[104]), "+f"(d[105]), "+f"(d[106]), "+f"(d[107]), "+f"(d[108]), "+f"(d[109]), "+f"(d[110]), "+f"(d[111]),
        "+f"(d[112]), "+f"(d[113]), "+f"(d[114]), "+f"(d[115]), "+f"(d[116]), "+f"(d[117]), "+f"(d[118]), "+f"(d[119]),
        "+f"(d[120]), "+f"(d[121]), "+f"(d[122]), "+f"(d[123]), "+f"(d[124]), "+f"(d[125]), "+f"(d[126]), "+f"(d[127])
      : "l"(da), "l"(db), "r"(scale_d));
}

__device__ __forceinline__ float sigmoid_mufu(float x) {
  float t, r;
  asm("ex2.approx.ftz.f32 %0, %1;" : "=f"(t) : "f"(-1.4426950408889634f * x));
  asm("rcp.approx.ftz.f32 %0, %1;" : "=f"(r) : "f"(1.0f + t));
  return r;
}
__device__ __forceinline__ void split4(float4 x, uint2& hi, uint2& lo) {
  __nv_bfloat162 h01 = __floats2bfloat162_rn(x.x, x.y), h23 = __floats2bfloat162_rn(x.z, x.w);
  float2 f01 = __bfloat1622float2(h01), f23 = __bfloat1622float2(h23);
  __nv_bfloat162 l01 = __floats2bfloat162_rn(x.x - f01.x, x.y - f01.y);
  __nv_bfloat162 l23 = __floats2bfloat162_rn(x.z - f23.x, x.w - f23.y);
  hi.x = *reinterpret_cast<uint32_t*>(&h01);
  hi.y = *reinterpret_cast<uint32_t*>(&h23);
  lo.x = *reinterpret_cast<uint32_t*>(&l01);
  lo.y = *reinterpret_cast<uint32_t*>(&l23);
}
__device__ __forceinline__ void split2(float a, float b, uint32_t& hi, uint32_t& lo) {
  __nv_bfloat162 h = __floats2bfloat162_rn(a, b);
  const float2 f = __bfloat1622float2(h);
  __nv_bfloat162 l = __floats2bfloat162_rn(a - f.x, b - f.y);
  hi = *reinterpret_cast<uint32_t*>(&h);
  lo = *reinterpret_cast<uint32_t*>(&l);
}
__device__ __forceinline__ uint32_t sw128_off(int r, int j) {
  return (uint32_t)((r >> 3) * 1024 + (r & 7) * 128 + ((j ^ (r & 7)) << 4));
}
__device__ __forceinline__ float quad_sum(float v) {
  v += __shfl_xor_sync(0xffffffffu, v, 1);
  return v + __shfl_xor_sync(0xffffffffu, v, 2);
}
__device__ __forceinline__ void swap_row_halves(float (&d)[128]) {
#pragma unroll
  for (int j = 0; j < 32; ++j) {
    const float x0 = d[4 * j], x1 = d[4 * j + 1];
    d[4 * j] = d[4 * j + 2];
    d[4 * j + 1] = d[4 * j + 3];
    d[4 * j + 2] = x0;
    d[4 * j + 3] = x1;
  }
}

enum {
  PH_TILES = 0,
  PH_TOTAL,
  PH_CONVERT,
  PH_G1_WAIT,
  PH_G1_MMA,
  PH_E1,
  PH_REDUCE,
  PH_LN,
  PH_G2_WAIT,
  PH_G2_MMA,
  PH_E4,
  PH_COUNT
};

template <int NWG, bool LIN, bool TIMED = false>
__device__ __forceinline__ void edge_layer_wg_body(const CUtensorMap& wmap, const TcParams& P) {
  using Cfg = TcCfg<NWG>;
  constexpr int NSTAGE = Cfg::NSTAGE;
  extern __shared__ unsigned char smem_raw[];
  unsigned char* smem = smem_raw + ((1024u - (smem_u32(smem_raw) & 1023u)) & 1023u);
  float* prm = reinterpret_cast<float*>(smem + Cfg::OFF_PRM);
  int* s_row = reinterpret_cast<int*>(smem + Cfg::OFF_ROW);
  const float** s_src = reinterpret_cast<const float**>(smem + Cfg::OFF_SRC);
  uint64_t* full = reinterpret_cast<uint64_t*>(smem + Cfg::OFF_BAR);
  uint64_t* empty = full + NSTAGE;

  const int warp = threadIdx.x >> 5, lane = threadIdx.x & 31;
  constexpr bool lin = LIN;
  const int loads_per_tile = (P.write_e ? 16 : 8) * NWG;

  if (threadIdx.x == 0) {
    for (int s = 0; s < NSTAGE; ++s) {
      mbar_init(&full[s], 1);
      mbar_init(&empty[s], 4);
    }
    asm volatile("fence.mbarrier_init.release.cluster;" ::: "memory");
    fence_proxy_async();
  }
  for (int i = threadIdx.x; i < H; i += Cfg::THREADS) {
    prm[i] = P.lp.ln_e_g[i];
    prm[H + i] = P.lp.ln_e_b[i];
    prm[2 * H + i] = P.tvec ? P.tvec[i] : 0.0f;
    prm[3 * H + i] = P.lp.ln_o_g[i];
    prm[4 * H + i] = P.lp.ln_o_b[i];
    prm[5 * H + i] = P.lp.b_O[i];
  }
  __syncthreads();
  const uint32_t smem_base = smem_u32(smem);

  if (warp >= 4 * NWG) {
    if constexpr (NWG == 2) asm volatile("setmaxnreg.dec.sync.aligned.u32 40;" ::: "memory");
    if (warp == 4 * NWG && lane == 0) {
      uint32_t u = 0;
      for (int tile = blockIdx.x; tile < P.n_tiles; tile += gridDim.x) {
        for (int i = 0; i < loads_per_tile; ++i, ++u) {
          const int s = u % NSTAGE;
          mbar_wait(&empty[s], ((u / NSTAGE) & 1) ^ 1, P.error_flag, 1);
          mbar_arrive_expect_tx(&full[s], TC_B_BYTES);
          const int row = (lin ? P.lin_w_row + (P.lin_nb == 4 ? (tile & 3) : 0) * W_MAT_ROWS
                               : P.w_row_base + (i >= 8 * NWG ? w_row_O(0) - w_row_C(0) : 0)) +
                          (i & 1) * W_LO_ROWS;
          tma_load_2d(smem_base + Cfg::OFF_B + s * TC_B_BYTES, &wmap, &full[s], ((i >> 1) & 3) * TC_KCH, row);
        }
      }
    }
    return;
  }

  if constexpr (NWG == 2) asm volatile("setmaxnreg.inc.sync.aligned.u32 232;" ::: "memory");
  const int wg = warp >> 2, wi = warp & 3, tid = threadIdx.x & 127;
  const int t4 = lane & 3;
  const int lr0 = wi * 16 + (lane >> 2);
  unsigned char* a_reg = smem + wg * TC_A_BYTES;
  const uint32_t a_base = smem_base + wg * TC_A_BYTES;
  float* msg = reinterpret_cast<float*>(a_reg);
  int* w_row = s_row + wg * WG_ROWS;
  const float** w_src = s_src + wg * WG_ROWS;
  auto wg_bar = [&] { asm volatile("bar.sync %0, 128;" ::"r"(1 + wg) : "memory"); };
  const int n_rows = lin ? P.lin_rows : P.g.E;
  uint32_t u = 0;
  float acc[128];

  auto turn_wait = [&] {
    if constexpr (NWG == 2) asm volatile("bar.sync %0, 256;" ::"r"(3 + wg) : "memory");
  };
  auto turn_pass = [&] {
    if constexpr (NWG == 2) asm volatile("bar.arrive %0, 256;" ::"r"(4 - wg) : "memory");
  };
  if (wg == 1) turn_pass();

  uint32_t t_mark = 0, t_start = 0;
  if constexpr (TIMED) t_start = t_mark = (uint32_t)clock();
  auto record = [&](int slot, uint32_t v) {
    if constexpr (TIMED) {
      if (tid == 0) atomicAdd(P.phase_cycles + slot, (unsigned long long)v);
    }
  };
  auto mark = [&](int slot) {
    if constexpr (TIMED) {
      const uint32_t now = (uint32_t)clock();
      record(slot, now - t_mark);
      t_mark = now;
    }
  };

  auto gemm = [&](int wait_slot, int mma_slot) {
    uint32_t waited = 0;
    turn_wait();
    if constexpr (TIMED) t_mark = (uint32_t)clock();
    acc_fence(acc);
    wgmma_fence();
    int s_prev = 0;
#pragma unroll
    for (int i = 0; i < 8; ++i, ++u) {
      const int s = u % NSTAGE;
      uint32_t w0 = 0;
      if constexpr (TIMED) w0 = (uint32_t)clock();
      mbar_wait(&full[s], (u / NSTAGE) & 1, P.error_flag, 2);
      if constexpr (TIMED) waited += (uint32_t)clock() - w0;
      const uint32_t b = smem_base + Cfg::OFF_B + s * TC_B_BYTES;
      const uint32_t ahi = a_base + (i >> 1) * 2 * TC_A_CHUNK, alo = ahi + TC_A_CHUNK;
#pragma unroll
      for (int ks = 0; ks < 4; ++ks) {
        const uint64_t db = wgmma_desc_sw128(b + ks * 32);
        wgmma_bf16(acc, wgmma_desc_sw128(ahi + ks * 32), db, (i | ks) ? 1u : 0u);
        if ((i & 1) == 0) wgmma_bf16(acc, wgmma_desc_sw128(alo + ks * 32), db, 1u);
      }
      wgmma_commit();
      if (i > 0) {
        wgmma_wait<1>();
        __syncwarp();
        if (lane == 0) mbar_arrive(&empty[s_prev]);
      }
      s_prev = s;
    }
    wgmma_wait<0>();
    acc_fence(acc);
    __syncwarp();
    if (lane == 0) mbar_arrive(&empty[s_prev]);
    turn_pass();
    if constexpr (TIMED) {
      const uint32_t now = (uint32_t)clock();
      record(wait_slot, waited);
      record(mma_slot, now - t_mark - waited);
      t_mark = now;
    }
  };

  for (int tile = blockIdx.x; tile < P.n_tiles; tile += gridDim.x) {
    record(PH_TILES, 1);
    const int row_tile = (lin && P.lin_nb == 4) ? (tile >> 2) : tile;
    const int s_base = row_tile * Cfg::TILE + wg * WG_ROWS;
    if (tid < WG_ROWS) {
      const int s = s_base + tid;
      const float* src = P.zero_row;
      int rw = -1;
      if (s < n_rows && lin) {
        src = P.lin_in + (size_t)s * H;
      } else if (s < n_rows) {
        rw = P.g.row[s];
        if (P.e_zero) src = P.zero_row;
        else if (P.xt_lut) src = P.lut + ((P.xt_lut[P.g.perm ? P.g.perm[s] : s] != 0.0f) ? H : 0);
        else src = P.e + (size_t)s * H;
      }
      w_row[tid] = rw;
      w_src[tid] = src;
    }
    wg_bar();

#pragma unroll 1
    for (int it0 = 0; it0 < 32; it0 += CONV_BATCH) {
      float4 x[CONV_BATCH];
#pragma unroll
      for (int q = 0; q < CONV_BATCH; ++q) {
        const int item = (it0 + q) * 128 + tid;
        x[q] = __ldcg(reinterpret_cast<const float4*>(w_src[item >> 6]) + (item & 63));
      }
#pragma unroll
      for (int q = 0; q < CONV_BATCH; ++q) {
        const int item = (it0 + q) * 128 + tid;
        const int rr = item >> 6, k4 = item & 63;
        uint2 hi, lo;
        split4(x[q], hi, lo);
        const uint32_t off = (k4 >> 4) * 2 * TC_A_CHUNK + sw128_off(rr, (k4 & 15) >> 1) + (k4 & 1) * 8;
        *reinterpret_cast<uint2*>(a_reg + off) = hi;
        *reinterpret_cast<uint2*>(a_reg + off + TC_A_CHUNK) = lo;
      }
    }
    fence_proxy_async();
    wg_bar();
    mark(PH_CONVERT);
    gemm(PH_G1_WAIT, PH_G1_MMA);

    const int sa = s_base + lr0, sb = sa + 8;
    const bool va = sa < n_rows, vb = sb < n_rows;
    if (lin || P.debug_acc) {
      const int nb = (lin && P.lin_nb == 4) ? (tile & 3) : 0;
      const int ostride = lin ? P.lin_nb * H : H;
      float* out = lin ? P.lin_out + nb * H : P.debug_acc;
#pragma unroll
      for (int h = 0; h < 2; ++h) {
        const int s = h ? sb : sa;
        if (!(h ? vb : va)) continue;
#pragma unroll
        for (int j = 0; j < 32; ++j) {
          const int c = 8 * j + 2 * t4;
          float2 o = make_float2(acc[4 * j + 2 * h], acc[4 * j + 2 * h + 1]);
          if (lin) {
            const float2 bb = __ldg(reinterpret_cast<const float2*>(P.lin_bias + nb * H + c));
            o.x += bb.x;
            o.y += bb.y;
          }
          __stcg(reinterpret_cast<float2*>(out + (size_t)s * ostride + c), o);
        }
      }
      continue;
    }

    const float* src_a = w_src[lr0];
    const float* src_b = w_src[lr0 + 8];
#pragma unroll 1
    for (int h = 0; h < 2; ++h) {
      const int s = h ? sb : sa;
      const bool v = h ? vb : va;
      const float* cp = P.uvab + (size_t)(v ? P.g.col[s] : 0) * 4 * H;
      const float* rp = P.uvab + (size_t)(v ? P.g.row[s] : 0) * 4 * H + 3 * H;
      const int r = lr0 + 8 * h;
#pragma unroll
      for (int j = 0; j < 32; ++j) {
        const int c = 8 * j + 2 * t4;
        const float2 ah = __ldg(reinterpret_cast<const float2*>(cp + 2 * H + c));
        const float2 vh = __ldg(reinterpret_cast<const float2*>(cp + H + c));
        const float2 bh = __ldg(reinterpret_cast<const float2*>(rp + c));
        const float x0 = (acc[4 * j] + ah.x) + bh.x;
        const float x1 = (acc[4 * j + 1] + ah.y) + bh.y;
        acc[4 * j] = x0;
        acc[4 * j + 1] = x1;
        *reinterpret_cast<float2*>(msg + r * H + (c ^ (8 * (r & 7)))) =
            make_float2(sigmoid_mufu(x0) * vh.x, sigmoid_mufu(x1) * vh.y);
      }
      swap_row_halves(acc);
    }
    wg_bar();
    mark(PH_E1);
    const bool amax = P.agg_mode == AGG_MAX;
    const float run0 = amax ? -INFINITY : 0.0f;
#pragma unroll 1
    for (int g2 = 0; g2 < WG_ROWS / GROUP; ++g2) {
      const int grp = (s_base >> 5) + g2;
      if (grp >= P.g.n_groups) break;
      const int first_node = P.g.grp_first[grp];
      const size_t pair_base = (size_t)P.g.grp_pair[grp];
      const int node = w_row[g2 * GROUP + lane];
      const int nxt = __shfl_down_sync(0xffffffffu, node, 1);
      const uint32_t ends = __ballot_sync(0xffffffffu, node >= 0 && (lane == GROUP - 1 || nxt != node));
#pragma unroll 1
      for (int cc = 0; cc < 2; ++cc) {
        const int c = tid + 128 * cc;
        float run = run0;
#pragma unroll 8
        for (int r = 0; r < GROUP; ++r) {
          const int lr = g2 * GROUP + r;
          const float m = msg[lr * H + (c ^ (8 * (lr & 7)))];
          run = amax ? fmaxf(run, m) : run + m;
          if ((ends >> r) & 1u) {
            P.partials[(pair_base + (size_t)(w_row[lr] - first_node)) * H + c] = run;
            run = run0;
          }
        }
      }
    }
    wg_bar();
    mark(PH_REDUCE);
    if (!P.write_e) continue;

#pragma unroll 1
    for (int h = 0; h < 2; ++h) {
      float sum = 0.f;
#pragma unroll
      for (int j = 0; j < 32; ++j) sum += acc[4 * j] + acc[4 * j + 1];
      float mean = quad_sum(sum) * (1.0f / H);
      float q = 0.f;
#pragma unroll
      for (int j = 0; j < 32; ++j) {
        const float d0 = acc[4 * j] - mean, d1 = acc[4 * j + 1] - mean;
        q = fmaf(d0, d0, fmaf(d1, d1, q));
      }
      float rstd = rsqrtf(quad_sum(q) * (1.0f / H) + LN_EPS);
      sum = 0.f;
#pragma unroll
      for (int j = 0; j < 32; ++j) {
        const int c = 8 * j + 2 * t4;
        const float2 g = *reinterpret_cast<const float2*>(prm + c);
        const float2 b = *reinterpret_cast<const float2*>(prm + H + c);
        const float2 t = *reinterpret_cast<const float2*>(prm + 2 * H + c);
        const float y0 = fmaxf(fmaf((acc[4 * j] - mean) * rstd, g.x, b.x), 0.0f) + t.x;
        const float y1 = fmaxf(fmaf((acc[4 * j + 1] - mean) * rstd, g.y, b.y), 0.0f) + t.y;
        acc[4 * j] = y0;
        acc[4 * j + 1] = y1;
        sum += y0 + y1;
      }
      mean = quad_sum(sum) * (1.0f / H);
      q = 0.f;
#pragma unroll
      for (int j = 0; j < 32; ++j) {
        const float d0 = acc[4 * j] - mean, d1 = acc[4 * j + 1] - mean;
        q = fmaf(d0, d0, fmaf(d1, d1, q));
      }
      rstd = rsqrtf(quad_sum(q) * (1.0f / H) + LN_EPS);
      const int r = lr0 + 8 * h;
#pragma unroll
      for (int j = 0; j < 32; ++j) {
        const int c = 8 * j + 2 * t4;
        const float2 g = *reinterpret_cast<const float2*>(prm + 3 * H + c);
        const float2 b = *reinterpret_cast<const float2*>(prm + 4 * H + c);
        const float z0 = fmaf((acc[4 * j] - mean) * rstd, g.x, b.x);
        const float z1 = fmaf((acc[4 * j + 1] - mean) * rstd, g.y, b.y);
        uint32_t hi, lo;
        split2(z0 * sigmoid_mufu(z0), z1 * sigmoid_mufu(z1), hi, lo);
        const uint32_t off = (j >> 3) * 2 * TC_A_CHUNK + sw128_off(r, j & 7) + 4 * t4;
        *reinterpret_cast<uint32_t*>(a_reg + off) = hi;
        *reinterpret_cast<uint32_t*>(a_reg + off + TC_A_CHUNK) = lo;
      }
      swap_row_halves(acc);
    }
    fence_proxy_async();
    wg_bar();
    mark(PH_LN);
    gemm(PH_G2_WAIT, PH_G2_MMA);

#pragma unroll
    for (int h = 0; h < 2; ++h) {
      if (!(h ? vb : va)) continue;
      const float* src = h ? src_b : src_a;
      float* dst = P.e + (size_t)(h ? sb : sa) * H;
#pragma unroll
      for (int j0 = 0; j0 < 32; j0 += E4_BATCH) {
        float2 ein[E4_BATCH];
#pragma unroll
        for (int q = 0; q < E4_BATCH; ++q) ein[q] = __ldcg(reinterpret_cast<const float2*>(src + 8 * (j0 + q) + 2 * t4));
#pragma unroll
        for (int q = 0; q < E4_BATCH; ++q) {
          const int j = j0 + q, c = 8 * j + 2 * t4;
          const float2 bo = *reinterpret_cast<const float2*>(prm + 5 * H + c);
          __stcg(reinterpret_cast<float2*>(dst + c),
                 make_float2((ein[q].x + acc[4 * j + 2 * h]) + bo.x, (ein[q].y + acc[4 * j + 2 * h + 1]) + bo.y));
        }
      }
    }
    mark(PH_E4);
  }
  if constexpr (TIMED) record(PH_TOTAL, (uint32_t)clock() - t_start);
}

__global__ void __launch_bounds__(TcCfg<2>::THREADS, 1)
k_edge_layer_wg2(const __grid_constant__ CUtensorMap wmap, const TcParams P) {
  edge_layer_wg_body<2, false>(wmap, P);
}
__global__ void __launch_bounds__(TcCfg<2>::THREADS, 1)
k_edge_layer_wg2_timed(const __grid_constant__ CUtensorMap wmap, const TcParams P) {
  edge_layer_wg_body<2, false, true>(wmap, P);
}
__global__ void __launch_bounds__(TcCfg<1>::THREADS, 1)
k_edge_layer_wg1(const __grid_constant__ CUtensorMap wmap, const TcParams P) {
  edge_layer_wg_body<1, false>(wmap, P);
}
__global__ void __launch_bounds__(TcCfg<2>::THREADS, 1)
k_linear_wg2(const __grid_constant__ CUtensorMap wmap, const TcParams P) {
  edge_layer_wg_body<2, true>(wmap, P);
}

struct TcState {
  std::string err;
  int num_sms = 0;
  CUtensorMap wmap;
  bool bound = false;
  float* zero_row = nullptr;
  int* error_flag = nullptr;
  int* error_host = nullptr;
  unsigned long long* phase_cycles = nullptr;

  TcState() = default;
  TcState(const TcState&) = delete;
  TcState& operator=(const TcState&) = delete;
  ~TcState() {
    if (zero_row) cudaFree(zero_row);
    if (error_host) cudaFreeHost(error_host);
    if (phase_cycles) cudaFree(phase_cycles);
  }
};

typedef CUresult (*PFN_encodeTiled)(CUtensorMap*, CUtensorMapDataType, cuuint32_t, void*, const cuuint64_t*,
                                    const cuuint64_t*, const cuuint32_t*, const cuuint32_t*, CUtensorMapInterleave,
                                    CUtensorMapSwizzle, CUtensorMapL2promotion, CUtensorMapFloatOOBfill);

inline int tc_init(TcState* st, int num_sms) {
  st->num_sms = num_sms;
  cudaError_t e = cudaFuncSetAttribute(k_edge_layer_wg2, cudaFuncAttributeMaxDynamicSharedMemorySize, TcCfg<2>::SMEM_ALLOC);
  if (e == cudaSuccess)
    e = cudaFuncSetAttribute(k_edge_layer_wg2_timed, cudaFuncAttributeMaxDynamicSharedMemorySize, TcCfg<2>::SMEM_ALLOC);
  if (e == cudaSuccess)
    e = cudaFuncSetAttribute(k_edge_layer_wg1, cudaFuncAttributeMaxDynamicSharedMemorySize, TcCfg<1>::SMEM_ALLOC);
  if (e == cudaSuccess)
    e = cudaFuncSetAttribute(k_linear_wg2, cudaFuncAttributeMaxDynamicSharedMemorySize, TcCfg<2>::SMEM_ALLOC);
  if (e != cudaSuccess) {
    st->err = std::string("cudaFuncSetAttribute: ") + cudaGetErrorString(e);
    return -2;
  }
  if ((e = cudaMalloc(&st->zero_row, H * sizeof(float))) != cudaSuccess ||
      (e = cudaMemset(st->zero_row, 0, H * sizeof(float))) != cudaSuccess ||
      (e = cudaMalloc(&st->phase_cycles, 32 * sizeof(unsigned long long))) != cudaSuccess ||
      (e = cudaMemset(st->phase_cycles, 0, 32 * sizeof(unsigned long long))) != cudaSuccess ||
      (e = cudaHostAlloc(&st->error_host, 4 * sizeof(int), cudaHostAllocMapped)) != cudaSuccess ||
      (e = cudaHostGetDevicePointer((void**)&st->error_flag, st->error_host, 0)) != cudaSuccess) {
    st->err = std::string("tc_init alloc: ") + cudaGetErrorString(e);
    return -2;
  }
  return 0;
}

inline int tc_bind_weights(TcState* st, const uint16_t* arena, int L) {
  void* fn = nullptr;
  cudaDriverEntryPointQueryResult qres;
  cudaError_t e = cudaGetDriverEntryPoint("cuTensorMapEncodeTiled", &fn, cudaEnableDefault, &qres);
  if (e != cudaSuccess || !fn || qres != cudaDriverEntryPointSuccess) {
    st->err = "cuTensorMapEncodeTiled entry point not available";
    cudaGetLastError();
    return -2;
  }
  cuuint64_t gdim[2] = {(cuuint64_t)H, (cuuint64_t)w_arena_rows(L)};
  cuuint64_t gstride[1] = {(cuuint64_t)H * sizeof(uint16_t)};
  cuuint32_t box[2] = {(cuuint32_t)TC_KCH, 256u};
  cuuint32_t estr[2] = {1u, 1u};
  CUresult r = ((PFN_encodeTiled)fn)(&st->wmap, CU_TENSOR_MAP_DATA_TYPE_BFLOAT16, 2, (void*)arena, gdim,
                                     gstride, box, estr, CU_TENSOR_MAP_INTERLEAVE_NONE, CU_TENSOR_MAP_SWIZZLE_128B,
                                     CU_TENSOR_MAP_L2_PROMOTION_L2_256B, CU_TENSOR_MAP_FLOAT_OOB_FILL_NONE);
  if (r != CUDA_SUCCESS) {
    st->err = "cuTensorMapEncodeTiled failed with CUresult " + std::to_string((int)r);
    return -2;
  }
  st->bound = true;
  return 0;
}

template <int NWG>
inline int tc_launch(TcState* st, void (*kernel)(CUtensorMap, TcParams), TcParams& P, int rows, int nb,
                     cudaStream_t stream) {
  if (!st->bound) {
    st->err = "weights not bound";
    return -1;
  }
  P.zero_row = st->zero_row; P.error_flag = st->error_flag; P.phase_cycles = st->phase_cycles;
  P.n_tiles = nb * ((rows + TcCfg<NWG>::TILE - 1) / TcCfg<NWG>::TILE);
  const int grid = P.n_tiles < st->num_sms ? P.n_tiles : st->num_sms;
  kernel<<<grid, TcCfg<NWG>::THREADS, TcCfg<NWG>::SMEM_ALLOC, stream>>>(st->wmap, P);
  const cudaError_t err = cudaGetLastError();
  if (err == cudaSuccess) return 0;
  st->err = std::string("launch: ") + cudaGetErrorString(err);
  return -2;
}

inline int tc_launch_edge_layer(TcState* st, int l, float* e, const float* uvab, float* partials, const GraphDev& g,
                                const LayerParams& lp, const float* tvec, int write_e, int e_zero, const float* xt_lut,
                                const float* lut, int agg_mode, int nwg, bool timed, float* debug_acc,
                                cudaStream_t stream) {
  TcParams P{};
  P.e = e; P.uvab = uvab; P.partials = partials; P.g = g; P.lp = lp; P.tvec = tvec;
  P.xt_lut = xt_lut; P.lut = lut; P.debug_acc = debug_acc;
  P.write_e = debug_acc ? 0 : write_e;
  P.e_zero = e_zero; P.agg_mode = agg_mode;
  P.w_row_base = w_row_C(l);
  if (nwg == 1) return tc_launch<1>(st, k_edge_layer_wg1, P, g.E, 1, stream);
  return tc_launch<2>(st, timed && !debug_acc ? k_edge_layer_wg2_timed : k_edge_layer_wg2, P, g.E, 1, stream);
}

inline int tc_launch_linear(TcState* st, const float* in, float* out, const float* bias, int rows, int nb, int w_row,
                            cudaStream_t stream) {
  TcParams P{};
  P.lin_in = in; P.lin_out = out; P.lin_bias = bias; P.lin_rows = rows; P.lin_nb = nb; P.lin_w_row = w_row;
  P.lp.ln_e_g = P.lp.ln_e_b = P.lp.ln_o_g = P.lp.ln_o_b = P.lp.b_O = st->zero_row;
  return tc_launch<2>(st, k_linear_wg2, P, rows, nb, stream);
}

}
```

### include/difusco_b200.h

```cpp
#ifndef DIFUSCO_B200_H_
#define DIFUSCO_B200_H_

#include <stdint.h>

#ifdef __cplusplus
extern "C" {
#endif

#define DFB_ABI_VERSION 2

enum {
  DFB_OK = 0,
  DFB_E_INVALID = -1,
  DFB_E_CUDA = -2,
  DFB_E_UNSUPPORTED = -3,
  DFB_E_NOMEM = -4
};

enum { DFB_TASK_TSP = 0, DFB_TASK_MIS = 1 };
enum { DFB_DIFFUSION_CATEGORICAL = 0, DFB_DIFFUSION_GAUSSIAN = 1 };
enum { DFB_EDGE_IMPL_TC = 0, DFB_EDGE_IMPL_FP32 = 1, DFB_EDGE_IMPL_TC1 = 2 };

typedef struct dfb_ctx dfb_ctx;

int dfb_abi_version(void);

int dfb_create(dfb_ctx** out, int device);
int dfb_destroy(dfb_ctx* ctx);
const char* dfb_last_error(const dfb_ctx* ctx);

int dfb_set_aggregation(dfb_ctx* ctx, int mode);

int dfb_set_edge_impl(dfb_ctx* ctx, int impl);

int dfb_load_weights(dfb_ctx* ctx, int n_layers, int hidden_dim, int out_channels,
                     int node_feature_only, int n_tensors, const char* const* names,
                     const float* const* tensors, const int64_t* numels);

int dfb_prepare_graph(dfb_ctx* ctx, const int64_t* edge_index, int64_t num_nodes, int64_t num_edges,
                      int gn_segments, void* stream);

int dfb_prepare_graph_instances(dfb_ctx* ctx, const int64_t* edge_index, int64_t num_nodes, int64_t num_edges,
                                int n_instances, const int64_t* node_ptr, void* stream);

int dfb_set_points(dfb_ctx* ctx, const float* points, void* stream);

int dfb_encoder_forward(dfb_ctx* ctx, const float* xt, float t, float* out, void* stream);

int dfb_denoise_step(dfb_ctx* ctx, int diffusion_type, const float* xt_in, float t,
                     const float* consts, int last, const float* uniforms, uint64_t seed,
                     int step_index, float* xt_out, float* p_out, float* net_out, void* stream);

int dfb_denoise(dfb_ctx* ctx, int diffusion_type, float* xt, int steps, const int32_t* t1,
                const float* consts, const int32_t* last_flags, const float* uniforms,
                uint64_t seed, void* stream);

int dfb_denoise_record(dfb_ctx* ctx, int diffusion_type, float* xt, int steps, const int32_t* t1,
                       const float* consts, const int32_t* last_flags, const float* uniforms, uint64_t seed,
                       int n_record, const int32_t* record_steps, float* rec_xt, float* rec_p, float* rec_out,
                       void* stream);

int dfb_set_graph_capture(dfb_ctx* ctx, int enabled);

int dfb_denoise_host(dfb_ctx* ctx, int diffusion_type, const float* points,
                     const int64_t* edge_index, int64_t num_nodes, int64_t num_edges,
                     int gn_segments, const float* xt0, int steps, const int32_t* t1,
                     const float* consts, const int32_t* last_flags, uint64_t seed,
                     float* heatmap_out, void* stream);

int dfb_knn_graph(dfb_ctx* ctx, const double* points, int64_t num_nodes, int k, int64_t node_offset,
                  int64_t* edge_index, void* stream);

int dfb_tsp_merge_sparse(const double* points, int64_t n, const float* heat, const int64_t* edge_index, int64_t E,
                         int mode, int64_t* tour, int64_t* merge_iterations);
int dfb_tsp_merge_order(int64_t n, const int64_t* order, int64_t count, int64_t* tour, int64_t* merge_iterations);

int dfb_two_opt(dfb_ctx* ctx, const double* points, int64_t n, int64_t* tours, int64_t batch, int64_t max_iterations,
                int64_t* iterations_out, void* stream);

int dfb_write_heatmap_txt(const char* path, int64_t n, const double* matrix);

int64_t dfb_launch_count(const dfb_ctx* ctx);

int dfb_profile_begin(dfb_ctx* ctx);
int dfb_profile_end(dfb_ctx* ctx, double* edge_kernel_ms, int64_t* edge_kernel_launches);

int dfb_debug_edge_gemm(dfb_ctx* ctx, int layer, const float* e_in, float* acc_out, void* stream);

int dfb_debug_gnn_layer(dfb_ctx* ctx, int layer, float t, float* h, float* e, void* stream);

int dfb_debug_phase_cycles(dfb_ctx* ctx, unsigned long long* out);

int dfb_set_phase_timing(dfb_ctx* ctx, int enabled);

int dfb_debug_watchdog(dfb_ctx* ctx, int* out);

#ifdef __cplusplus
}
#endif
#endif
```

Before: 20.46.

## Add four-consumer-warpgroup edge kernel splitting output columns across warpgroups

Adds an NWG=4 variant of the warp-specialized edge-layer kernel and makes it the default TC path. Four consumer warpgroups split each 128-row tile into two row blocks and two column halves, so each warpgroup uses an m64n128 wgmma with 64 accumulators. LayerNorm statistics are exchanged between column halves through shared memory and named barriers. The intent is to raise consumer parallelism and lower per-thread register pressure, at the cost of extra cross-warpgroup synchronization, a lower register cap (112), and smaller load batches.

Result: faster. 20.71 (median of 6 runs) (+1.2%).

```diff
diff --git a/difusco_b200/_cabi.py b/difusco_b200/_cabi.py
--- a/difusco_b200/_cabi.py
+++ b/difusco_b200/_cabi.py
@@ -8,7 +8,7 @@
 
 DFB_OK, DFB_E_INVALID, DFB_E_CUDA, DFB_E_UNSUPPORTED, DFB_E_NOMEM = 0, -1, -2, -3, -4
 CATEGORICAL, GAUSSIAN = 0, 1
-EDGE_IMPL_TC, EDGE_IMPL_FP32, EDGE_IMPL_TC1 = 0, 1, 2
+EDGE_IMPL_TC, EDGE_IMPL_FP32, EDGE_IMPL_TC1, EDGE_IMPL_TC2 = 0, 1, 2, 3
 AGGREGATION = {"sum": 0, "mean": 1, "max": 2}
 
 SYMBOLS = [
diff --git a/difusco_b200/csrc/dfb_api.cu b/difusco_b200/csrc/dfb_api.cu
--- a/difusco_b200/csrc/dfb_api.cu
+++ b/difusco_b200/csrc/dfb_api.cu
@@ -233,7 +233,8 @@
 
 extern "C" int dfb_set_edge_impl(dfb_ctx* ctx, int impl) {
   if (!ctx) return DFB_E_INVALID;
-  if (impl != DFB_EDGE_IMPL_TC && impl != DFB_EDGE_IMPL_FP32 && impl != DFB_EDGE_IMPL_TC1) FAIL(ctx, DFB_E_INVALID, "unknown edge impl %d", impl);
+  if (impl != DFB_EDGE_IMPL_TC && impl != DFB_EDGE_IMPL_FP32 && impl != DFB_EDGE_IMPL_TC1 && impl != DFB_EDGE_IMPL_TC2)
+    FAIL(ctx, DFB_E_INVALID, "unknown edge impl %d", impl);
   ctx->edge_impl = impl;
   return DFB_OK;
 }
@@ -595,7 +596,8 @@
 
 struct EdgeImpl { bool fp32; int nwg; };
 static EdgeImpl edge_impl(const dfb_ctx* ctx) {
-  return {ctx->edge_impl == DFB_EDGE_IMPL_FP32, ctx->edge_impl == DFB_EDGE_IMPL_TC1 ? 1 : 2};
+  const int nwg = ctx->edge_impl == DFB_EDGE_IMPL_TC1 ? 1 : ctx->edge_impl == DFB_EDGE_IMPL_TC2 ? 2 : 4;
+  return {ctx->edge_impl == DFB_EDGE_IMPL_FP32, nwg};
 }
 
 static int linear_rows(dfb_ctx* ctx, const float* X, const float* Wt, int w_row, const float* b, float* Y, int R, int N,
diff --git a/difusco_b200/csrc/edge_layer_tc.cuh b/difusco_b200/csrc/edge_layer_tc.cuh
--- a/difusco_b200/csrc/edge_layer_tc.cuh
+++ b/difusco_b200/csrc/edge_layer_tc.cuh
@@ -31,15 +31,23 @@
 
 template <int NWG>
 struct TcCfg {
-  static_assert(NWG == 1 || NWG == 2, "one or two consumer warpgroups");
-  static constexpr int TILE = NWG * WG_ROWS;
+  static_assert(NWG == 1 || NWG == 2 || NWG == 4, "one, two or four consumer warpgroups");
+  static constexpr int NRB = NWG == 1 ? 1 : 2;
+  static constexpr int NC = NWG / NRB;
+  static constexpr int NCOL = H / NC;
+  static constexpr int ACC = NCOL / 2;
+  static constexpr int TILE = NRB * WG_ROWS;
   static constexpr int THREADS = (NWG + 1) * 128;
   static constexpr int NSTAGE = (NWG == 1) ? 3 : 2;
-  static constexpr int OFF_B = NWG * TC_A_BYTES;
+  static constexpr int CONV_B = NC == 1 ? CONV_BATCH : 4;
+  static constexpr int E4_B = NC == 1 ? E4_BATCH : 8;
+  static constexpr int E1_B = 8;
+  static constexpr int OFF_B = NRB * TC_A_BYTES;
   static constexpr int OFF_PRM = OFF_B + NSTAGE * TC_B_BYTES;
   static constexpr int OFF_ROW = OFF_PRM + 6 * H * 4;
   static constexpr int OFF_SRC = OFF_ROW + TILE * 4;
-  static constexpr int OFF_BAR = OFF_SRC + TILE * 8;
+  static constexpr int OFF_LNX = OFF_SRC + TILE * 8;
+  static constexpr int OFF_BAR = OFF_LNX + (NC == 2 ? NRB * 2 * 128 * 4 : 0);
   static constexpr int SMEM_BYTES = OFF_BAR + 2 * NSTAGE * 8;
   static constexpr int SMEM_ALLOC = SMEM_BYTES + 1024;
   static_assert(SMEM_ALLOC <= 232448, "shared memory budget (227 KB per block)");
@@ -118,9 +126,10 @@
 __device__ __forceinline__ void wgmma_commit() { asm volatile("wgmma.commit_group.sync.aligned;" ::: "memory"); }
 template <int N>
 __device__ __forceinline__ void wgmma_wait() { asm volatile("wgmma.wait_group.sync.aligned %0;" ::"n"(N) : "memory"); }
-__device__ __forceinline__ void acc_fence(float (&d)[128]) {
-#pragma unroll
-  for (int i = 0; i < 128; ++i) asm volatile("" : "+f"(d[i])::"memory");
+template <int N>
+__device__ __forceinline__ void acc_fence(float (&d)[N]) {
+#pragma unroll
+  for (int i = 0; i < N; ++i) asm volatile("" : "+f"(d[i])::"memory");
 }
 __device__ __forceinline__ void wgmma_bf16(float (&d)[128], uint64_t da, uint64_t db, uint32_t scale_d) {
   asm volatile(
@@ -153,6 +162,25 @@
         "+f"(d[120]), "+f"(d[121]), "+f"(d[122]), "+f"(d[123]), "+f"(d[124]), "+f"(d[125]), "+f"(d[126]), "+f"(d[127])
       : "l"(da), "l"(db), "r"(scale_d));
 }
+__device__ __forceinline__ void wgmma_bf16(float (&d)[64], uint64_t da, uint64_t db, uint32_t scale_d) {
+  asm volatile(
+      "{\n .reg .pred p;\n setp.ne.b32 p, %66, 0;\n"
+      "wgmma.mma_async.sync.aligned.m64n128k16.f32.bf16.bf16 "
+      "{%0, %1, %2, %3, %4, %5, %6, %7, %8, %9, %10, %11, %12, %13, %14, %15, "
+      "%16, %17, %18, %19, %20, %21, %22, %23, %24, %25, %26, %27, %28, %29, %30, %31, "
+      "%32, %33, %34, %35, %36, %37, %38, %39, %40, %41, %42, %43, %44, %45, %46, %47, "
+      "%48, %49, %50, %51, %52, %53, %54, %55, %56, %57, %58, %59, %60, %61, %62, %63}, "
+      "%64, %65, p, 1, 1, 0, 0;\n}"
+      : "+f"(d[0]), "+f"(d[1]), "+f"(d[2]), "+f"(d[3]), "+f"(d[4]), "+f"(d[5]), "+f"(d[6]), "+f"(d[7]),
+        "+f"(d[8]), "+f"(d[9]), "+f"(d[10]), "+f"(d[11]), "+f"(d[12]), "+f"(d[13]), "+f"(d[14]), "+f"(d[15]),
+        "+f"(d[16]), "+f"(d[17]), "+f"(d[18]), "+f"(d[19]), "+f"(d[20]), "+f"(d[21]), "+f"(d[22]), "+f"(d[23]),
+        "+f"(d[24]), "+f"(d[25]), "+f"(d[26]), "+f"(d[27]), "+f"(d[28]), "+f"(d[29]), "+f"(d[30]), "+f"(d[31]),
+        "+f"(d[32]), "+f"(d[33]), "+f"(d[34]), "+f"(d[35]), "+f"(d[36]), "+f"(d[37]), "+f"(d[38]), "+f"(d[39]),
+        "+f"(d[40]), "+f"(d[41]), "+f"(d[42]), "+f"(d[43]), "+f"(d[44]), "+f"(d[45]), "+f"(d[46]), "+f"(d[47]),
+        "+f"(d[48]), "+f"(d[49]), "+f"(d[50]), "+f"(d[51]), "+f"(d[52]), "+f"(d[53]), "+f"(d[54]), "+f"(d[55]),
+        "+f"(d[56]), "+f"(d[57]), "+f"(d[58]), "+f"(d[59]), "+f"(d[60]), "+f"(d[61]), "+f"(d[62]), "+f"(d[63])
+      : "l"(da), "l"(db), "r"(scale_d));
+}
 
 __device__ __forceinline__ float sigmoid_mufu(float x) {
   float t, r;
@@ -184,14 +212,29 @@
   v += __shfl_xor_sync(0xffffffffu, v, 1);
   return v + __shfl_xor_sync(0xffffffffu, v, 2);
 }
-__device__ __forceinline__ void swap_row_halves(float (&d)[128]) {
-#pragma unroll
-  for (int j = 0; j < 32; ++j) {
+template <int N>
+__device__ __forceinline__ void swap_row_halves(float (&d)[N]) {
+#pragma unroll
+  for (int j = 0; j < N / 4; ++j) {
     const float x0 = d[4 * j], x1 = d[4 * j + 1];
     d[4 * j] = d[4 * j + 2];
     d[4 * j + 1] = d[4 * j + 3];
     d[4 * j + 2] = x0;
     d[4 * j + 3] = x1;
+  }
+}
+
+template <int B, int N>
+__device__ __forceinline__ void rotate_pairs(float (&d)[N]) {
+  constexpr int NP = N / 2, JN = N / 4;
+  float t[N];
+#pragma unroll
+  for (int i = 0; i < N; ++i) t[i] = d[i];
+#pragma unroll
+  for (int k = 0; k < NP; ++k) {
+    const int ks = (k + B) % NP;
+    d[4 * (k % JN) + 2 * (k / JN)] = t[4 * (ks % JN) + 2 * (ks / JN)];
+    d[4 * (k % JN) + 2 * (k / JN) + 1] = t[4 * (ks % JN) + 2 * (ks / JN) + 1];
   }
 }
 
@@ -213,7 +256,8 @@
 template <int NWG, bool LIN, bool TIMED = false>
 __device__ __forceinline__ void edge_layer_wg_body(const CUtensorMap& wmap, const TcParams& P) {
   using Cfg = TcCfg<NWG>;
-  constexpr int NSTAGE = Cfg::NSTAGE;
+  constexpr int NSTAGE = Cfg::NSTAGE, NRB = Cfg::NRB, NC = Cfg::NC, NCOL = Cfg::NCOL;
+  constexpr int JN = Cfg::ACC / 4;
   extern __shared__ unsigned char smem_raw[];
   unsigned char* smem = smem_raw + ((1024u - (smem_u32(smem_raw) & 1023u)) & 1023u);
   float* prm = reinterpret_cast<float*>(smem + Cfg::OFF_PRM);
@@ -224,12 +268,12 @@
 
   const int warp = threadIdx.x >> 5, lane = threadIdx.x & 31;
   constexpr bool lin = LIN;
-  const int loads_per_tile = (P.write_e ? 16 : 8) * NWG;
+  const int loads_per_tile = (P.write_e ? 16 : 8) * NRB;
 
   if (threadIdx.x == 0) {
     for (int s = 0; s < NSTAGE; ++s) {
       mbar_init(&full[s], 1);
-      mbar_init(&empty[s], 4);
+      mbar_init(&empty[s], 4 * NC);
     }
     asm volatile("fence.mbarrier_init.release.cluster;" ::: "memory");
     fence_proxy_async();
@@ -247,6 +291,7 @@
 
   if (warp >= 4 * NWG) {
     if constexpr (NWG == 2) asm volatile("setmaxnreg.dec.sync.aligned.u32 40;" ::: "memory");
+    if constexpr (NWG == 4) asm volatile("setmaxnreg.dec.sync.aligned.u32 24;" ::: "memory");
     if (warp == 4 * NWG && lane == 0) {
       uint32_t u = 0;
       for (int tile = blockIdx.x; tile < P.n_tiles; tile += gridDim.x) {
@@ -255,7 +300,7 @@
           mbar_wait(&empty[s], ((u / NSTAGE) & 1) ^ 1, P.error_flag, 1);
           mbar_arrive_expect_tx(&full[s], TC_B_BYTES);
           const int row = (lin ? P.lin_w_row + (P.lin_nb == 4 ? (tile & 3) : 0) * W_MAT_ROWS
-                               : P.w_row_base + (i >= 8 * NWG ? w_row_O(0) - w_row_C(0) : 0)) +
+                               : P.w_row_base + (i >= 8 * NRB ? w_row_O(0) - w_row_C(0) : 0)) +
                           (i & 1) * W_LO_ROWS;
           tma_load_2d(smem_base + Cfg::OFF_B + s * TC_B_BYTES, &wmap, &full[s], ((i >> 1) & 3) * TC_KCH, row);
         }
@@ -265,32 +310,61 @@
   }
 
   if constexpr (NWG == 2) asm volatile("setmaxnreg.inc.sync.aligned.u32 232;" ::: "memory");
+  if constexpr (NWG == 4) asm volatile("setmaxnreg.inc.sync.aligned.u32 112;" ::: "memory");
   const int wg = warp >> 2, wi = warp & 3, tid = threadIdx.x & 127;
+  const int rb = NC == 1 ? wg : (wg & 1), cs = NC == 1 ? 0 : (wg >> 1);
+  const int col0 = cs * NCOL;
   const int t4 = lane & 3;
   const int lr0 = wi * 16 + (lane >> 2);
-  unsigned char* a_reg = smem + wg * TC_A_BYTES;
-  const uint32_t a_base = smem_base + wg * TC_A_BYTES;
+  unsigned char* a_reg = smem + rb * TC_A_BYTES;
+  const uint32_t a_base = smem_base + rb * TC_A_BYTES;
   float* msg = reinterpret_cast<float*>(a_reg);
-  int* w_row = s_row + wg * WG_ROWS;
-  const float** w_src = s_src + wg * WG_ROWS;
-  auto wg_bar = [&] { asm volatile("bar.sync %0, 128;" ::"r"(1 + wg) : "memory"); };
+  int* w_row = s_row + rb * WG_ROWS;
+  const float** w_src = s_src + rb * WG_ROWS;
+  auto wg_bar = [&] { asm volatile("bar.sync %0, %1;" ::"r"(1 + rb), "n"(128 * NC) : "memory"); };
   const int n_rows = lin ? P.lin_rows : P.g.E;
   uint32_t u = 0;
-  float acc[128];
+  float acc[Cfg::ACC];
 
   auto turn_wait = [&] {
-    if constexpr (NWG == 2) asm volatile("bar.sync %0, 256;" ::"r"(3 + wg) : "memory");
+    if constexpr (NRB == 2) asm volatile("bar.sync %0, %1;" ::"r"(3 + rb), "n"(256 * NC) : "memory");
   };
   auto turn_pass = [&] {
-    if constexpr (NWG == 2) asm volatile("bar.arrive %0, 256;" ::"r"(4 - wg) : "memory");
+    if constexpr (NRB == 2) asm volatile("bar.arrive %0, %1;" ::"r"(4 - rb), "n"(256 * NC) : "memory");
   };
-  if (wg == 1) turn_pass();
+  if (rb == 1) turn_pass();
+
+  float* lnx = reinterpret_cast<float*>(smem + Cfg::OFF_LNX) + rb * 256;
+  auto chain_start = [&]() -> float {
+    if constexpr (NC == 2) {
+      if (cs == 1) {
+        asm volatile("bar.sync %0, 256;" ::"r"(5 + 2 * rb) : "memory");
+        return lnx[tid];
+      }
+    }
+    return 0.0f;
+  };
+  auto chain_total = [&](float v) -> float {
+    if constexpr (NC == 2) {
+      if (cs == 0) {
+        lnx[tid] = v;
+        asm volatile("bar.arrive %0, 256;" ::"r"(5 + 2 * rb) : "memory");
+        asm volatile("bar.sync %0, 256;" ::"r"(6 + 2 * rb) : "memory");
+        return lnx[128 + tid];
+      }
+      v = quad_sum(v);
+      lnx[128 + tid] = v;
+      asm volatile("bar.arrive %0, 256;" ::"r"(6 + 2 * rb) : "memory");
+      return v;
+    }
+    return quad_sum(v);
+  };
 
   uint32_t t_mark = 0, t_start = 0;
   if constexpr (TIMED) t_start = t_mark = (uint32_t)clock();
   auto record = [&](int slot, uint32_t v) {
     if constexpr (TIMED) {
-      if (tid == 0) atomicAdd(P.phase_cycles + slot, (unsigned long long)v);
+      if (tid == 0 && cs == 0) atomicAdd(P.phase_cycles + slot, (unsigned long long)v);
     }
   };
   auto mark = [&](int slot) {
@@ -308,28 +382,32 @@
     acc_fence(acc);
     wgmma_fence();
     int s_prev = 0;
-#pragma unroll
-    for (int i = 0; i < 8; ++i, ++u) {
-      const int s = u % NSTAGE;
-      uint32_t w0 = 0;
-      if constexpr (TIMED) w0 = (uint32_t)clock();
-      mbar_wait(&full[s], (u / NSTAGE) & 1, P.error_flag, 2);
-      if constexpr (TIMED) waited += (uint32_t)clock() - w0;
-      const uint32_t b = smem_base + Cfg::OFF_B + s * TC_B_BYTES;
-      const uint32_t ahi = a_base + (i >> 1) * 2 * TC_A_CHUNK, alo = ahi + TC_A_CHUNK;
-#pragma unroll
-      for (int ks = 0; ks < 4; ++ks) {
-        const uint64_t db = wgmma_desc_sw128(b + ks * 32);
-        wgmma_bf16(acc, wgmma_desc_sw128(ahi + ks * 32), db, (i | ks) ? 1u : 0u);
-        if ((i & 1) == 0) wgmma_bf16(acc, wgmma_desc_sw128(alo + ks * 32), db, 1u);
-      }
-      wgmma_commit();
-      if (i > 0) {
-        wgmma_wait<1>();
-        __syncwarp();
-        if (lane == 0) mbar_arrive(&empty[s_prev]);
-      }
-      s_prev = s;
+#pragma unroll (NC == 1 ? 4 : 1)
+    for (int kc = 0; kc < 4; ++kc) {
+#pragma unroll
+      for (int ii = 0; ii < 2; ++ii, ++u) {
+        const int i = 2 * kc + ii;
+        const int s = u % NSTAGE;
+        uint32_t w0 = 0;
+        if constexpr (TIMED) w0 = (uint32_t)clock();
+        mbar_wait(&full[s], (u / NSTAGE) & 1, P.error_flag, 2);
+        if constexpr (TIMED) waited += (uint32_t)clock() - w0;
+        const uint32_t b = smem_base + Cfg::OFF_B + s * TC_B_BYTES + col0 * 128;
+        const uint32_t ahi = a_base + kc * 2 * TC_A_CHUNK, alo = ahi + TC_A_CHUNK;
+#pragma unroll
+        for (int ks = 0; ks < 4; ++ks) {
+          const uint64_t db = wgmma_desc_sw128(b + ks * 32);
+          wgmma_bf16(acc, wgmma_desc_sw128(ahi + ks * 32), db, (i | ks) ? 1u : 0u);
+          if (ii == 0) wgmma_bf16(acc, wgmma_desc_sw128(alo + ks * 32), db, 1u);
+        }
+        wgmma_commit();
+        if (NC == 2 || i > 0) {
+          wgmma_wait<1>();
+          __syncwarp();
+          if (lane == 0 && i > 0) mbar_arrive(&empty[s_prev]);
+        }
+        s_prev = s;
+      }
     }
     wgmma_wait<0>();
     acc_fence(acc);
@@ -347,8 +425,8 @@
   for (int tile = blockIdx.x; tile < P.n_tiles; tile += gridDim.x) {
     record(PH_TILES, 1);
     const int row_tile = (lin && P.lin_nb == 4) ? (tile >> 2) : tile;
-    const int s_base = row_tile * Cfg::TILE + wg * WG_ROWS;
-    if (tid < WG_ROWS) {
+    const int s_base = row_tile * Cfg::TILE + rb * WG_ROWS;
+    if (tid < WG_ROWS && cs == 0) {
       const int s = s_base + tid;
       const float* src = P.zero_row;
       int rw = -1;
@@ -365,18 +443,19 @@
     }
     wg_bar();
 
+    constexpr int KQ_LOG = NC == 1 ? 6 : 5, KQ = 1 << KQ_LOG;
 #pragma unroll 1
-    for (int it0 = 0; it0 < 32; it0 += CONV_BATCH) {
-      float4 x[CONV_BATCH];
-#pragma unroll
-      for (int q = 0; q < CONV_BATCH; ++q) {
+    for (int it0 = 0; it0 < 32 / NC; it0 += Cfg::CONV_B) {
+      float4 x[Cfg::CONV_B];
+#pragma unroll
+      for (int q = 0; q < Cfg::CONV_B; ++q) {
         const int item = (it0 + q) * 128 + tid;
-        x[q] = __ldcg(reinterpret_cast<const float4*>(w_src[item >> 6]) + (item & 63));
-      }
-#pragma unroll
-      for (int q = 0; q < CONV_BATCH; ++q) {
+        x[q] = __ldcg(reinterpret_cast<const float4*>(w_src[item >> KQ_LOG]) + cs * KQ + (item & (KQ - 1)));
+      }
+#pragma unroll
+      for (int q = 0; q < Cfg::CONV_B; ++q) {
         const int item = (it0 + q) * 128 + tid;
-        const int rr = item >> 6, k4 = item & 63;
+        const int rr = item >> KQ_LOG, k4 = cs * KQ + (item & (KQ - 1));
         uint2 hi, lo;
         split4(x[q], hi, lo);
         const uint32_t off = (k4 >> 4) * 2 * TC_A_CHUNK + sw128_off(rr, (k4 & 15) >> 1) + (k4 & 1) * 8;
@@ -400,8 +479,8 @@
         const int s = h ? sb : sa;
         if (!(h ? vb : va)) continue;
 #pragma unroll
-        for (int j = 0; j < 32; ++j) {
-          const int c = 8 * j + 2 * t4;
+        for (int j = 0; j < JN; ++j) {
+          const int c = col0 + 8 * j + 2 * t4;
           float2 o = make_float2(acc[4 * j + 2 * h], acc[4 * j + 2 * h + 1]);
           if (lin) {
             const float2 bb = __ldg(reinterpret_cast<const float2*>(P.lin_bias + nb * H + c));
@@ -416,27 +495,61 @@
 
     const float* src_a = w_src[lr0];
     const float* src_b = w_src[lr0 + 8];
+    if constexpr (NC == 2) {
+      wg_bar();
+      const float* cps[2];
+      const float* rps[2];
+#pragma unroll
+      for (int h = 0; h < 2; ++h) {
+        const int s = h ? sb : sa;
+        const bool v = h ? vb : va;
+        cps[h] = P.uvab + (size_t)(v ? P.g.col[s] : 0) * 4 * H;
+        rps[h] = P.uvab + (size_t)(v ? P.g.row[s] : 0) * 4 * H + 3 * H;
+      }
 #pragma unroll 1
-    for (int h = 0; h < 2; ++h) {
-      const int s = h ? sb : sa;
-      const bool v = h ? vb : va;
-      const float* cp = P.uvab + (size_t)(v ? P.g.col[s] : 0) * 4 * H;
-      const float* rp = P.uvab + (size_t)(v ? P.g.row[s] : 0) * 4 * H + 3 * H;
-      const int r = lr0 + 8 * h;
-#pragma unroll
-      for (int j = 0; j < 32; ++j) {
-        const int c = 8 * j + 2 * t4;
-        const float2 ah = __ldg(reinterpret_cast<const float2*>(cp + 2 * H + c));
-        const float2 vh = __ldg(reinterpret_cast<const float2*>(cp + H + c));
-        const float2 bh = __ldg(reinterpret_cast<const float2*>(rp + c));
-        const float x0 = (acc[4 * j] + ah.x) + bh.x;
-        const float x1 = (acc[4 * j + 1] + ah.y) + bh.y;
-        acc[4 * j] = x0;
-        acc[4 * j + 1] = x1;
-        *reinterpret_cast<float2*>(msg + r * H + (c ^ (8 * (r & 7)))) =
-            make_float2(sigmoid_mufu(x0) * vh.x, sigmoid_mufu(x1) * vh.y);
-      }
-      swap_row_halves(acc);
+      for (int k0 = 0; k0 < 2 * JN; k0 += Cfg::E1_B) {
+        const int h = k0 / JN, jb = k0 % JN;
+        const float* cp = h ? cps[1] : cps[0];
+        const float* rp = h ? rps[1] : rps[0];
+        const int r = lr0 + 8 * h;
+#pragma unroll
+        for (int q = 0; q < Cfg::E1_B; ++q) {
+          const int c = col0 + 8 * (jb + q) + 2 * t4;
+          const float2 ah = __ldg(reinterpret_cast<const float2*>(cp + 2 * H + c));
+          const float2 vh = __ldg(reinterpret_cast<const float2*>(cp + H + c));
+          const float2 bh = __ldg(reinterpret_cast<const float2*>(rp + c));
+          const float x0 = (acc[4 * q] + ah.x) + bh.x;
+          const float x1 = (acc[4 * q + 1] + ah.y) + bh.y;
+          acc[4 * q] = x0;
+          acc[4 * q + 1] = x1;
+          *reinterpret_cast<float2*>(msg + r * H + (c ^ (8 * (r & 7)))) =
+              make_float2(sigmoid_mufu(x0) * vh.x, sigmoid_mufu(x1) * vh.y);
+        }
+        rotate_pairs<Cfg::E1_B>(acc);
+      }
+    } else {
+#pragma unroll 1
+      for (int h = 0; h < 2; ++h) {
+        const int s = h ? sb : sa;
+        const bool v = h ? vb : va;
+        const float* cp = P.uvab + (size_t)(v ? P.g.col[s] : 0) * 4 * H;
+        const float* rp = P.uvab + (size_t)(v ? P.g.row[s] : 0) * 4 * H + 3 * H;
+        const int r = lr0 + 8 * h;
+#pragma unroll
+        for (int j = 0; j < JN; ++j) {
+          const int c = col0 + 8 * j + 2 * t4;
+          const float2 ah = __ldg(reinterpret_cast<const float2*>(cp + 2 * H + c));
+          const float2 vh = __ldg(reinterpret_cast<const float2*>(cp + H + c));
+          const float2 bh = __ldg(reinterpret_cast<const float2*>(rp + c));
+          const float x0 = (acc[4 * j] + ah.x) + bh.x;
+          const float x1 = (acc[4 * j + 1] + ah.y) + bh.y;
+          acc[4 * j] = x0;
+          acc[4 * j + 1] = x1;
+          *reinterpret_cast<float2*>(msg + r * H + (c ^ (8 * (r & 7)))) =
+              make_float2(sigmoid_mufu(x0) * vh.x, sigmoid_mufu(x1) * vh.y);
+        }
+        swap_row_halves(acc);
+      }
     }
     wg_bar();
     mark(PH_E1);
@@ -452,8 +565,8 @@
       const int nxt = __shfl_down_sync(0xffffffffu, node, 1);
       const uint32_t ends = __ballot_sync(0xffffffffu, node >= 0 && (lane == GROUP - 1 || nxt != node));
 #pragma unroll 1
-      for (int cc = 0; cc < 2; ++cc) {
-        const int c = tid + 128 * cc;
+      for (int cc = 0; cc < 2 / NC; ++cc) {
+        const int c = col0 + tid + 128 * cc;
         float run = run0;
 #pragma unroll 8
         for (int r = 0; r < GROUP; ++r) {
@@ -473,21 +586,21 @@
 
 #pragma unroll 1
     for (int h = 0; h < 2; ++h) {
-      float sum = 0.f;
-#pragma unroll
-      for (int j = 0; j < 32; ++j) sum += acc[4 * j] + acc[4 * j + 1];
-      float mean = quad_sum(sum) * (1.0f / H);
-      float q = 0.f;
-#pragma unroll
-      for (int j = 0; j < 32; ++j) {
+      float sum = chain_start();
+#pragma unroll
+      for (int j = 0; j < JN; ++j) sum += acc[4 * j] + acc[4 * j + 1];
+      float mean = chain_total(sum) * (1.0f / H);
+      float q = chain_start();
+#pragma unroll
+      for (int j = 0; j < JN; ++j) {
         const float d0 = acc[4 * j] - mean, d1 = acc[4 * j + 1] - mean;
         q = fmaf(d0, d0, fmaf(d1, d1, q));
       }
-      float rstd = rsqrtf(quad_sum(q) * (1.0f / H) + LN_EPS);
+      float rstd = rsqrtf(chain_total(q) * (1.0f / H) + LN_EPS);
       sum = 0.f;
 #pragma unroll
-      for (int j = 0; j < 32; ++j) {
-        const int c = 8 * j + 2 * t4;
+      for (int j = 0; j < JN; ++j) {
+        const int c = col0 + 8 * j + 2 * t4;
         const float2 g = *reinterpret_cast<const float2*>(prm + c);
         const float2 b = *reinterpret_cast<const float2*>(prm + H + c);
         const float2 t = *reinterpret_cast<const float2*>(prm + 2 * H + c);
@@ -495,27 +608,33 @@
         const float y1 = fmaxf(fmaf((acc[4 * j + 1] - mean) * rstd, g.y, b.y), 0.0f) + t.y;
         acc[4 * j] = y0;
         acc[4 * j + 1] = y1;
-        sum += y0 + y1;
-      }
-      mean = quad_sum(sum) * (1.0f / H);
-      q = 0.f;
-#pragma unroll
-      for (int j = 0; j < 32; ++j) {
+        if constexpr (NC == 1) sum += y0 + y1;
+      }
+      if constexpr (NC == 2) {
+        sum = chain_start();
+#pragma unroll
+        for (int j = 0; j < JN; ++j) sum += acc[4 * j] + acc[4 * j + 1];
+      }
+      mean = chain_total(sum) * (1.0f / H);
+      q = chain_start();
+#pragma unroll
+      for (int j = 0; j < JN; ++j) {
         const float d0 = acc[4 * j] - mean, d1 = acc[4 * j + 1] - mean;
         q = fmaf(d0, d0, fmaf(d1, d1, q));
       }
-      rstd = rsqrtf(quad_sum(q) * (1.0f / H) + LN_EPS);
+      rstd = rsqrtf(chain_total(q) * (1.0f / H) + LN_EPS);
       const int r = lr0 + 8 * h;
 #pragma unroll
-      for (int j = 0; j < 32; ++j) {
-        const int c = 8 * j + 2 * t4;
+      for (int j = 0; j < JN; ++j) {
+        const int c = col0 + 8 * j + 2 * t4;
         const float2 g = *reinterpret_cast<const float2*>(prm + 3 * H + c);
         const float2 b = *reinterpret_cast<const float2*>(prm + 4 * H + c);
         const float z0 = fmaf((acc[4 * j] - mean) * rstd, g.x, b.x);
         const float z1 = fmaf((acc[4 * j + 1] - mean) * rstd, g.y, b.y);
         uint32_t hi, lo;
         split2(z0 * sigmoid_mufu(z0), z1 * sigmoid_mufu(z1), hi, lo);
-        const uint32_t off = (j >> 3) * 2 * TC_A_CHUNK + sw128_off(r, j & 7) + 4 * t4;
+        const int jk = (col0 >> 3) + j;
+        const uint32_t off = (jk >> 3) * 2 * TC_A_CHUNK + sw128_off(r, jk & 7) + 4 * t4;
         *reinterpret_cast<uint32_t*>(a_reg + off) = hi;
         *reinterpret_cast<uint32_t*>(a_reg + off + TC_A_CHUNK) = lo;
       }
@@ -532,13 +651,14 @@
       const float* src = h ? src_b : src_a;
       float* dst = P.e + (size_t)(h ? sb : sa) * H;
 #pragma unroll
-      for (int j0 = 0; j0 < 32; j0 += E4_BATCH) {
-        float2 ein[E4_BATCH];
-#pragma unroll
-        for (int q = 0; q < E4_BATCH; ++q) ein[q] = __ldcg(reinterpret_cast<const float2*>(src + 8 * (j0 + q) + 2 * t4));
-#pragma unroll
-        for (int q = 0; q < E4_BATCH; ++q) {
-          const int j = j0 + q, c = 8 * j + 2 * t4;
+      for (int j0 = 0; j0 < JN; j0 += Cfg::E4_B) {
+        float2 ein[Cfg::E4_B];
+#pragma unroll
+        for (int q = 0; q < Cfg::E4_B; ++q)
+          ein[q] = __ldcg(reinterpret_cast<const float2*>(src + col0 + 8 * (j0 + q) + 2 * t4));
+#pragma unroll
+        for (int q = 0; q < Cfg::E4_B; ++q) {
+          const int j = j0 + q, c = col0 + 8 * j + 2 * t4;
           const float2 bo = *reinterpret_cast<const float2*>(prm + 5 * H + c);
           __stcg(reinterpret_cast<float2*>(dst + c),
                  make_float2((ein[q].x + acc[4 * j + 2 * h]) + bo.x, (ein[q].y + acc[4 * j + 2 * h + 1]) + bo.y));
@@ -550,6 +670,14 @@
   if constexpr (TIMED) record(PH_TOTAL, (uint32_t)clock() - t_start);
 }
 
+__global__ void __launch_bounds__(TcCfg<4>::THREADS, 1)
+k_edge_layer_wg4(const __grid_constant__ CUtensorMap wmap, const TcParams P) {
+  edge_layer_wg_body<4, false>(wmap, P);
+}
+__global__ void __launch_bounds__(TcCfg<4>::THREADS, 1)
+k_edge_layer_wg4_timed(const __grid_constant__ CUtensorMap wmap, const TcParams P) {
+  edge_layer_wg_body<4, false, true>(wmap, P);
+}
 __global__ void __launch_bounds__(TcCfg<2>::THREADS, 1)
 k_edge_layer_wg2(const __grid_constant__ CUtensorMap wmap, const TcParams P) {
   edge_layer_wg_body<2, false>(wmap, P);
@@ -593,7 +721,11 @@
 
 inline int tc_init(TcState* st, int num_sms) {
   st->num_sms = num_sms;
-  cudaError_t e = cudaFuncSetAttribute(k_edge_layer_wg2, cudaFuncAttributeMaxDynamicSharedMemorySize, TcCfg<2>::SMEM_ALLOC);
+  cudaError_t e = cudaFuncSetAttribute(k_edge_layer_wg4, cudaFuncAttributeMaxDynamicSharedMemorySize, TcCfg<4>::SMEM_ALLOC);
+  if (e == cudaSuccess)
+    e = cudaFuncSetAttribute(k_edge_layer_wg4_timed, cudaFuncAttributeMaxDynamicSharedMemorySize, TcCfg<4>::SMEM_ALLOC);
+  if (e == cudaSuccess)
+    e = cudaFuncSetAttribute(k_edge_layer_wg2, cudaFuncAttributeMaxDynamicSharedMemorySize, TcCfg<2>::SMEM_ALLOC);
   if (e == cudaSuccess)
     e = cudaFuncSetAttribute(k_edge_layer_wg2_timed, cudaFuncAttributeMaxDynamicSharedMemorySize, TcCfg<2>::SMEM_ALLOC);
   if (e == cudaSuccess)
@@ -667,8 +799,10 @@
   P.write_e = debug_acc ? 0 : write_e;
   P.e_zero = e_zero; P.agg_mode = agg_mode;
   P.w_row_base = w_row_C(l);
+  timed = timed && !debug_acc;
   if (nwg == 1) return tc_launch<1>(st, k_edge_layer_wg1, P, g.E, 1, stream);
-  return tc_launch<2>(st, timed && !debug_acc ? k_edge_layer_wg2_timed : k_edge_layer_wg2, P, g.E, 1, stream);
+  if (nwg == 2) return tc_launch<2>(st, timed ? k_edge_layer_wg2_timed : k_edge_layer_wg2, P, g.E, 1, stream);
+  return tc_launch<4>(st, timed ? k_edge_layer_wg4_timed : k_edge_layer_wg4, P, g.E, 1, stream);
 }
 
 inline int tc_launch_linear(TcState* st, const float* in, float* out, const float* bias, int rows, int nb, int w_row,
diff --git a/include/difusco_b200.h b/include/difusco_b200.h
--- a/include/difusco_b200.h
+++ b/include/difusco_b200.h
@@ -19,7 +19,7 @@
 
 enum { DFB_TASK_TSP = 0, DFB_TASK_MIS = 1 };
 enum { DFB_DIFFUSION_CATEGORICAL = 0, DFB_DIFFUSION_GAUSSIAN = 1 };
-enum { DFB_EDGE_IMPL_TC = 0, DFB_EDGE_IMPL_FP32 = 1, DFB_EDGE_IMPL_TC1 = 2 };
+enum { DFB_EDGE_IMPL_TC = 0, DFB_EDGE_IMPL_FP32 = 1, DFB_EDGE_IMPL_TC1 = 2, DFB_EDGE_IMPL_TC2 = 3 };
 
 typedef struct dfb_ctx dfb_ctx;
 
```
